# nubomedia/NUBOMEDIA-VCA

Measured on NVIDIA B200. Metric: 1080p face-cascade frames/s, higher is better.
Workload: dtype u8 pixels, int32/u32 integrals, f32 features, f64 stage sums

## Files before the change

nubomedia-vca_b200/csrc/context.cu:

```cuda
#include <math.h>
#include <stdio.h>
#include <stdlib.h>
#include <string.h>

#include <algorithm>
#include <atomic>

#include "internal.h"

#define NV_VERSION_STR "nubovca-b200 0.1 (sm_100a)"
#define CAND_CAP 8192
#define CAND_CAP_GROUPED 65536
#define CAND_CAP_RAW 131072

extern "C" const char *nv_version(void) { return NV_VERSION_STR; }

extern "C" int nv_device_count(void)
{
    int n = 0;
    if (cudaGetDeviceCount(&n) != cudaSuccess) { cudaGetLastError(); return 0; }
    return n;
}

extern "C" int nv_cascade_load(const char *xml_path, nv_cascade **out)
// ... 89 lines not shown
    }
    if (leaves) for (int i = 0; i <= nn; i++) leaves[i] = c->h.leaves[l0 + i];
    return NV_OK;
}

extern "C" int nv_debug_cascade_feature(const nv_cascade *c, int feature, int rects12[12], float weights3[3], int *tilted)
{
    if (!c || feature < 0 || feature >= (int)c->h.feat_tilted.size() || !rects12 || !weights3) { nv_set_error("bad argument"); return NV_ERR_ARG; }
    for (int i = 0; i < 12; i++) rects12[i] = c->h.feat_rect[(size_t)feature * 12 + i];
    for (int i = 0; i < 3; i++) weights3[i] = c->h.feat_weight[(size_t)feature * 3 + i];
    if (tilted) *tilted = c->h.feat_tilted[feature];
    return NV_OK;
}

extern "C" int nv_debug_cascade_subset(const nv_cascade *c, int node, int subset8[8])
{
    if (!c || !subset8 || !c->h.lbp || node < 0 || (size_t)node * 8 + 8 > c->h.node_subset.size()) { nv_set_error("bad argument"); return NV_ERR_ARG; }
    for (int k = 0; k < 8; k++) subset8[k] = c->h.node_subset[(size_t)node * 8 + k];
    return NV_OK;
}

extern "C" void nv_cascade_free(nv_cascade *c)
{
    if (!c) return;
    for (auto &kv : c->d_stumps) { cudaSetDevice(kv.first); cudaFree(kv.second); }
    for (auto &kv : c->d_meta) { cudaSetDevice(kv.first); cudaFree(kv.second); }
    for (auto &kv : c->d_tail) { cudaSetDevice(kv.first); cudaFree(kv.second); }
    for (auto &kv : c->d_tail_base) { cudaSetDevice(kv.first); cudaFree(kv.second); }
    for (auto &kv : c->d_gen) {
        cudaSetDevice(kv.first);
        cudaFree((void *)kv.second.tree); cudaFree((void *)kv.second.node); cudaFree((void *)kv.second.leaf); cudaFree((void *)kv.second.feat);
        cudaFree((void *)kv.second.subset);
    }
    delete c;
}

static int cascade_on_device(nv_cascade *c, int gpu, cudaStream_t st, const DevStump **stumps, const DevCascade **meta)
{
    std::lock_guard<std::mutex> lk(c->mu);
    (void)st;
    if (c->d_stumps.find(gpu) == c->d_stumps.end()) {
        std::vector<void *> owned;
        struct Guard {
            std::vector<void *> &v; bool keep = false;
            ~Guard() { if (!keep) for (void *p : v) cudaFree(p); }
        } guard{owned};
        auto upload = [&](const void *src, size_t bytes, void **out) -> int {
            void *d = nullptr;
            NV_CUDA(cudaMalloc(&d, bytes ? bytes : 1));
            owned.push_back(d);
            if (bytes) NV_CUDA(cudaMemcpy(d, src, bytes, cudaMemcpyHostToDevice));
            *out = d;
            return NV_OK;
        };
        int rc;
        void *ds = nullptr, *dm = nullptr, *dtree = nullptr, *dnode = nullptr, *dleaf = nullptr, *dfeat = nullptr, *dt = nullptr, *db = nullptr, *dsub = nullptr;
        if ((rc = upload(c->stumps.data(), c->stumps.size() * sizeof(DevStump), &ds)) != NV_OK) return rc;
        if ((rc = upload(&c->meta, sizeof(DevCascade), &dm)) != NV_OK) return rc;
        if (c->h.general) {
            const HostCascade &h = c->h;
            std::vector<int2> trees(h.tree_nnodes.size());
            std::vector<int4> nodes(h.node_feat.size());
            std::vector<GenFeat> feats(h.feat_tilted.size());
            int n0 = 0, l0 = 0;
            for (size_t t = 0; t < trees.size(); t++) { trees[t] = make_int2(n0, l0); n0 += h.tree_nnodes[t]; l0 += h.tree_nnodes[t] + 1; }
            for (size_t i = 0; i < nodes.size(); i++) {
                int tb; memcpy(&tb, &h.node_thr[i], 4);
                nodes[i] = make_int4(h.node_feat[i], tb, h.node_left[i], h.node_right[i]);
            }
            for (size_t f = 0; f < feats.size(); f++) {
                GenFeat &g = feats[f];
                memset(&g, 0, sizeof g);
                for (int k = 0; k < 3; k++) {
                    const int *r = &h.feat_rect[f * 12 + 4 * k];
                    g.r[k] = (uint32_t)r[0] | ((uint32_t)r[1] << 8) | ((uint32_t)r[2] << 16) | ((uint32_t)r[3] << 24);
                    g.w[k] = h.feat_weight[f * 3 + k];
                }
                g.tilted = h.feat_tilted[f];
            }
            if ((rc = upload(trees.data(), trees.size() * sizeof(int2), &dtree)) != NV_OK) return rc;
            if ((rc = upload(nodes.data(), nodes.size() * sizeof(int4), &dnode)) != NV_OK) return rc;
            if ((rc = upload(h.leaves.data(), h.leaves.size() * sizeof(float), &dleaf)) != NV_OK) return rc;
            if ((rc = upload(feats.data(), feats.size() * sizeof(GenFeat), &dfeat)) != NV_OK) return rc;
            if (h.lbp && (rc = upload(h.node_subset.data(), h.node_subset.size() * sizeof(int), &dsub)) != NV_OK) return rc;
        }
        if (c->tail_fast) {
            if ((rc = upload(c->tail_stumps.data(), c->tail_stumps.size() * sizeof(TailStump), &dt)) != NV_OK) return rc;
            if ((rc = upload(c->tail_base.data(), c->tail_base.size() * sizeof(double), &db)) != NV_OK) return rc;
        }
        guard.keep = true;
        if (c->h.general) c->d_gen[gpu] = GenModel{(int2 *)dtree, (int4 *)dnode, (float *)dleaf, (GenFeat *)dfeat, (uint32_t *)dsub};
        if (c->tail_fast) { c->d_tail[gpu] = (TailStump *)dt; c->d_tail_base[gpu] = (double *)db; }
        c->d_meta[gpu] = (DevCascade *)dm;
        c->d_stumps[gpu] = (DevStump *)ds;
    }
    *stumps = c->d_stumps[gpu]; *meta = c->d_meta[gpu];
    return NV_OK;
}

template <typename T>
static int ensure(T **p, size_t *cap, size_t need, bool zero = false)
{
    if (*p && *cap >= need) return NV_OK;
    if (*p) { NV_CUDA(cudaFree(*p)); *p = nullptr; }
    size_t n = need + need / 8 + 64;
    NV_CUDA(cudaMalloc(p, n * sizeof(T)));
    if (zero) NV_CUDA(cudaMemset(*p, 0, n * sizeof(T)));
    *cap = n;
    return NV_OK;
}

static int alloc_candidates(nv_ctx *c, int cap, bool with_adj)
{
    cudaFree(c->d_cand); cudaFree(c->d_cand_sorted); cudaFree(c->d_cand_rects); cudaFree(c->d_adj); cudaFree(c->d_result);
    cudaFree(c->d_cand_w); cudaFree(c->d_cls_wmax);
    cudaFreeHost(c->h_result);
    c->d_cand = c->d_cand_sorted = nullptr; c->d_cand_rects = nullptr; c->d_adj = nullptr; c->d_result = c->h_result = nullptr;
    c->d_cand_w = nullptr; c->d_cls_wmax = nullptr;
    c->cand_cap = cap; c->result_cap = cap; c->adj_cap = 0; c->epoch++;
    NV_CUDA(cudaMalloc(&c->d_cand, (size_t)cap * sizeof(uint32_t)));
    NV_CUDA(cudaMalloc(&c->d_cand_sorted, (size_t)cap * sizeof(uint32_t)));
    NV_CUDA(cudaMalloc(&c->d_cand_rects, (size_t)cap * sizeof(int4)));
    NV_CUDA(cudaMalloc(&c->d_cand_w, (size_t)cap * sizeof(double)));
    NV_CUDA(cudaMalloc(&c->d_cls_wmax, (size_t)cap * sizeof(unsigned long long)));
    const size_t acap = std::min<size_t>((size_t)cap, NV_GROUP_UF_MIN);
    size_t adj_words = (with_adj ? acap * ((acap + 31) / 32) : 0) + 8 * (size_t)cap;
    NV_CUDA(cudaMalloc(&c->d_adj, adj_words * sizeof(uint32_t)));
    c->adj_cap = with_adj ? cap : 0;
    c->d_grp = reinterpret_cast<int *>(c->d_adj + (adj_words - 8 * (size_t)cap));
    size_t rbytes = sizeof(ResultHeader) + (size_t)c->result_cap * (sizeof(nv_rect) + sizeof(double) + sizeof(int));
    NV_CUDA(cudaMalloc(&c->d_result, rbytes));
    NV_CUDA(cudaMallocHost(&c->h_result, rbytes));
    memset(c->h_result, 0, sizeof(ResultHeader));
    return NV_OK;
}

extern "C" int nv_ctx_create(int gpu, int max_width, int max_height, nv_ctx **out)
{
    if (!out || max_width <= 0 || max_height <= 0 || max_width > 16384 || max_height > 16384) {
        nv_set_error("nv_ctx_create: bad argument");
        return NV_ERR_ARG;
    }
    *out = nullptr;
    int ndev = nv_device_count();
    if (ndev <= 0) { nv_set_error("no CUDA device visible: libnubovca has no CPU path"); return NV_ERR_NO_DEVICE; }
    if (gpu < 0 || gpu >= ndev) { nv_set_error("gpu ordinal %d out of range (0..%d)", gpu, ndev - 1); return NV_ERR_ARG; }
    NV_CUDA(cudaSetDevice(gpu));
    nv_ctx *c = new nv_ctx();
    c->gpu = gpu; c->max_w = max_width; c->max_h = max_height;
    int rc = [&]() -> int {
        NV_CUDA(cudaStreamCreateWithFlags(&c->stream, cudaStreamNonBlocking));
        NV_CUDA(cudaEventCreateWithFlags(&c->ev_done, cudaEventDisableTiming));
        NV_CUDA(cudaStreamCreateWithFlags(&c->stream2, cudaStreamNonBlocking));
        for (int i = 0; i < 2; i++) {
            NV_CUDA(cudaEventCreateWithFlags(&c->ev_fork[i], cudaEventDisableTiming));
            NV_CUDA(cudaEventCreateWithFlags(&c->ev_join[i], cudaEventDisableTiming));
        }
        c->frame_cap = (size_t)max_width * max_height * 4 + 4096;
        NV_CUDA(cudaMallocHost(&c->h_frame, c->frame_cap));
        NV_CUDA(cudaMalloc(&c->d_frame, c->frame_cap));
        c->gray_cap = (size_t)max_width * max_height + 256;
        NV_CUDA(cudaMalloc(&c->d_gray, c->gray_cap));
        NV_CUDA(cudaMalloc(&c->d_hist, 260 * sizeof(int)));
        NV_CUDA(cudaMemset(c->d_hist, 0, 260 * sizeof(int)));
        NV_CUDA(cudaMalloc(&c->d_lut, 512));
        uint8_t ident[256];
        for (int i = 0; i < 256; i++) ident[i] = (uint8_t)i;
        NV_CUDA(cudaMemcpy(c->d_lut + 256, ident, 256, cudaMemcpyHostToDevice));
        c->slots = new PlanSlot[NV_PLAN_SLOTS];
        c->ps = &c->slots[0];
        for (int i = 0; i < NV_PLAN_SLOTS; i++) NV_CUDA(cudaMalloc(&c->slots[i].d_plan, sizeof(PlanDev)));
        NV_CUDA(cudaMalloc(&c->d_counters, 16 * sizeof(int)));
        NV_CUDA(cudaMemset(c->d_counters, 0, 16 * sizeof(int)));
        NV_CUDA(cudaMalloc(&c->d_deepq, NV_DEEPQ_CAP * sizeof(uint2)));
        return alloc_candidates(c, CAND_CAP, true);
    }();
    if (rc != NV_OK) { nv_ctx_destroy(c); return rc; }
    *out = c;
    return NV_OK;
}

static void batch_free(nv_ctx::Batch &b);

extern "C" void nv_ctx_destroy(nv_ctx *c)
{
    if (!c) return;
    cudaSetDevice(c->gpu);
    if (c->stream) cudaStreamSynchronize(c->stream);
    cudaFreeHost(c->h_frame); cudaFree(c->d_frame); cudaFree(c->d_gray); cudaFree(c->d_hist); cudaFree(c->d_lut);
    cudaFree(c->d_aux); for (auto &e : c->rtabs) cudaFree(e.d); cudaFree(c->d_sum);
    if (c->slots) {
        for (int i = 0; i < NV_PLAN_SLOTS; i++) {
            PlanSlot &sl = c->slots[i];
            cudaFree(sl.d_plan); cudaFree(sl.d_ptab); cudaFree(sl.d_maps);
            if (sl.dexec) cudaGraphExecDestroy(sl.dexec);
        }
        delete[] c->slots;
    }
    cudaFree(c->d_sq); cudaFree(c->d_pyr); cudaFree(c->d_tilt); cudaFree(c->d_vnf); cudaFree(c->d_depth);
    cudaFree(c->d_bits_ok); cudaFree(c->d_queue); cudaFree(c->d_queue2); cudaFree(c->d_deepq); cudaFree(c->d_counters); cudaFree(c->d_cand);
    cudaFree(c->d_cand_sorted); cudaFree(c->d_cand_rects); cudaFree(c->d_adj); cudaFree(c->d_result);
    cudaFree(c->d_cand_w); cudaFree(c->d_cls_wmax);
    cudaFreeHost(c->h_result);
    cudaFree(c->d_trk_prev); cudaFree(c->d_trk_hist); cudaFree(c->d_trk_scratch); cudaFreeHost(c->h_trk);
    if (c->gexec) cudaGraphExecDestroy(c->gexec);
    if (c->bexec) cudaGraphExecDestroy(c->bexec);
    batch_free(c->b);
    if (c->ev_done) cudaEventDestroy(c->ev_done);
    for (int i = 0; i < 2; i++) { if (c->ev_fork[i]) cudaEventDestroy(c->ev_fork[i]); if (c->ev_join[i]) cudaEventDestroy(c->ev_join[i]); }
    if (c->stream2) cudaStreamDestroy(c->stream2);
    for (int i = 0; i <= NV_NUM_STAGES; i++) if (c->prof_ev[i]) cudaEventDestroy(c->prof_ev[i]);
    if (c->stream) cudaStreamDestroy(c->stream);
    cudaGetLastError();
    delete c;
}

extern "C" int nv_ctx_set_scores(nv_ctx *ctx, int on)
{
    if (!ctx) { nv_set_error("null ctx"); return NV_ERR_ARG; }
    ctx->scores = on ? 1 : 0;
    return NV_OK;
}

extern "C" int nv_get_scores(nv_ctx *ctx, int *neighbors, double *level_weights, int cap, int *n)
{
    if (!ctx) { nv_set_error("null ctx"); return NV_ERR_ARG; }
    if (!ctx->scores_ready || ctx->batch_last) { nv_set_error("no collected call with scores on"); return NV_ERR_STATE; }
    const int total = reinterpret_cast<const ResultHeader *>(ctx->h_result)->n_out, m = std::min(total, std::max(cap, 0));
    const uint8_t *w = ctx->h_result + sizeof(ResultHeader) + (size_t)ctx->result_cap * sizeof(nv_rect);
    const uint8_t *nb = w + (size_t)ctx->result_cap * sizeof(double);
    if (level_weights && m > 0) memcpy(level_weights, w, (size_t)m * sizeof(double));
    if (neighbors && m > 0) memcpy(neighbors, nb, (size_t)m * sizeof(int));
    if (n) *n = m;
    if (total > cap) { nv_set_error("%d rectangles, caller capacity %d", total, cap); return NV_ERR_CAPACITY; }
    return NV_OK;
}

extern "C" int nv_ctx_set_debug(nv_ctx *ctx, int debug)
{
    if (!ctx) { nv_set_error("null ctx"); return NV_ERR_ARG; }
    ctx->debug = debug ? 1 : 0;
    ctx->epoch++;
    for (int i = 0; ctx->slots && i < NV_PLAN_SLOTS; i++) ctx->slots[i].plan_valid = false;
    return NV_OK;
}

static const char *k_stage_names[NV_NUM_STAGES] = {"face_prep", "hist_lut", "pyramid_rowscan", "integral_colscan",
                                                   "cascade_stage0", "cascade_tiles", "cascade_tail", "group_rectangles"};
extern "C" const char *nv_stage_name(int slot) { return slot >= 0 && slot < NV_NUM_STAGES ? k_stage_names[slot] : ""; }

static inline void prof_mark(nv_ctx *ctx, int idx)
{
    if (!ctx->profile) return;
    cudaStreamCaptureStatus cs = cudaStreamCaptureStatusNone;
    cudaStreamIsCapturing(ctx->stream, &cs);
    if (cs == cudaStreamCaptureStatusActive) cudaEventRecordWithFlags(ctx->prof_ev[idx], ctx->stream, cudaEventRecordExternal);
    else cudaEventRecord(ctx->prof_ev[idx], ctx->stream);
    ctx->prof_set[idx] = true;
}

extern "C" int nv_ctx_set_profile(nv_ctx *ctx, int on)
{
    if (!ctx) { nv_set_error("null ctx"); return NV_ERR_ARG; }
    NV_CUDA(cudaSetDevice(ctx->gpu));
    if (on && !ctx->prof_ev[0])
        for (int i = 0; i <= NV_NUM_STAGES; i++) NV_CUDA(cudaEventCreate(&ctx->prof_ev[i]));
    if (ctx->profile != (on ? 1 : 0)) ctx->epoch++;
    ctx->profile = on ? 1 : 0;
    return NV_OK;
}

extern "C" int nv_ctx_get_stage_times(nv_ctx *ctx, float *ms, int cap, int *n)
{
    if (!ctx || !ms) { nv_set_error("null argument"); return NV_ERR_ARG; }
    if (!ctx->profile || ctx->pending) { nv_set_error("profiling off or call still pending"); return NV_ERR_STATE; }
    if (ctx->batch_last) { nv_set_error("stage times describe single calls: the last call was a batch"); return NV_ERR_STATE; }
    NV_CUDA(cudaSetDevice(ctx->gpu));
    int m = std::min(cap, NV_NUM_STAGES);
    for (int i = 0; i < m; i++) {
        ms[i] = 0.f;
        if (ctx->prof_set[i] && ctx->prof_set[i + 1]) NV_CUDA(cudaEventElapsedTime(&ms[i], ctx->prof_ev[i], ctx->prof_ev[i + 1]));
    }
    if (n) *n = m;
    return NV_OK;
}

extern "C" int nv_event_create(void **ev)
{
    if (!ev) { nv_set_error("null argument"); return NV_ERR_ARG; }
    cudaEvent_t e;
    NV_CUDA(cudaEventCreate(&e));
    *ev = e;
    return NV_OK;
}
extern "C" int nv_event_record(nv_ctx *ctx, void *ev)
{
    if (!ctx || !ev) { nv_set_error("null argument"); return NV_ERR_ARG; }
    NV_CUDA(cudaSetDevice(ctx->gpu));
    NV_CUDA(cudaEventRecord((cudaEvent_t)ev, ctx->stream));
    return NV_OK;
}
extern "C" int nv_event_elapsed_ms(void *e0, void *e1, float *ms)
{
    if (!e0 || !e1 || !ms) { nv_set_error("null argument"); return NV_ERR_ARG; }
    NV_CUDA(cudaEventSynchronize((cudaEvent_t)e1));
    NV_CUDA(cudaEventElapsedTime(ms, (cudaEvent_t)e0, (cudaEvent_t)e1));
    return NV_OK;
}
extern "C" void nv_event_destroy(void *ev) { if (ev) cudaEventDestroy((cudaEvent_t)ev); }

static inline int cv_round(double v) { return (int)lrint(v); }
static inline int cv_roundf(float v) { return (int)lrintf(v); }
static inline int align_up(int v, int a) { return (v + a - 1) / a * a; }

static void exact_coefs(int ssize, int dsize, int2 *tab, int lead, int total)
{
    double scale = 1.0 / ((double)dsize / ssize);
    for (int k = 0; k < total; k++) tab[k] = make_int2(0, 0);
    for (int d = 0; d < dsize; d++) {
        double f = scale * (d + 0.5) - 0.5;
        int i = (int)floor(f);
        if (i >= 0 && i < ssize - 1) tab[lead + d] = make_int2(i, cv_round((f - i) * 256.0));
        else if (i < 0) tab[lead + d] = make_int2(0, 0);
        else tab[lead + d] = ssize >= 2 ? make_int2(ssize - 2, 256) : make_int2(0, 0);
    }
}

static int ensure_plan(nv_ctx *ctx, const nv_cascade *casc, int W, int H, const nv_detect_params *p)
{
    if (!(p->scale_factor > 1.0)) {
        nv_set_error("scale_factor must be > 1 (got %g): OpenCV would never terminate", p->scale_factor);
        return NV_ERR_ARG;
    }
    PlanKey key;
    key.W = W; key.H = H; key.win_w = casc->h.win_w; key.win_h = casc->h.win_h;
    key.min_w = p->min_w; key.min_h = p->min_h; key.max_w = p->max_w; key.max_h = p->max_h; key.sf = p->scale_factor;
    key.casc = casc->uid;
    if (ctx->ps->plan_valid && key == ctx->ps->pkey) { ctx->ps->last_use = ++ctx->use_clock; return NV_OK; }
    PlanSlot *victim = nullptr;
    for (int i = 0; i < NV_PLAN_SLOTS; i++) {
        PlanSlot &sl = ctx->slots[i];
        if (sl.plan_valid && key == sl.pkey) {
            ctx->ps = &sl;
            sl.last_use = ++ctx->use_clock;
            if (sl.buf_gen != ctx->buf_gen) { sl.tp_casc = 0; sl.buf_gen = ctx->buf_gen; }
            return NV_OK;
        }
        if (!victim || (!sl.plan_valid && victim->plan_valid) || (sl.plan_valid == victim->plan_valid && sl.last_use < victim->last_use))
            victim = &sl;
    }
    ctx->ps = victim;
    ctx->ps->plan_valid = false;
    ctx->ps->last_use = ++ctx->use_clock;

    PlanDev &P = ctx->ps->plan;
    memset(&P, 0, sizeof P);
    P.W = W; P.H = H; P.win_w = key.win_w; P.win_h = key.win_h;
    int max_w = p->max_w, max_h = p->max_h;
    if (max_w == 0 || max_h == 0) { max_w = W; max_h = H; }
    std::vector<float> scales;
    for (double f = 1;; f *= p->scale_factor) {
        int ww = cv_round(key.win_w * f), wh = cv_round(key.win_h * f);
        if (ww > max_w || wh > max_h || ww > W || wh > H) break;
        if (ww < p->min_w || wh < p->min_h) continue;
        scales.push_back((float)f);
        if (scales.size() > 4096) break;
    }
    int nstripes = 1;
    long long iofs = 0, wofs = 0, bofs = 0, tofs = 0, pofs = 0;
    int nl = 0;
    for (size_t k = 0; k < scales.size(); k++) {
        float sc = scales[k];
        int lw = cv_roundf((float)W / sc), lh = cv_roundf((float)H / sc);
        int rx = lw + 1 - key.win_w, ry = lh + 1 - key.win_h;
        if (k == 0) nstripes = std::max((std::max(rx, 0) + 31) / 32, 1);
        if (rx <= 0 || ry <= 0) continue;
        int ystep = sc >= 2.f ? 1 : 2;
        int stripe = std::max((ry / ystep + nstripes - 1) / nstripes, 1) * ystep;
        long long lim = (long long)stripe * nstripes;
        if (lim < ry) ry = (int)lim;
        if (nl >= NV_MAX_LEVELS) { nv_set_error("more than %d pyramid levels", NV_MAX_LEVELS); return NV_ERR_CAPACITY; }
        LevelDesc &L = P.lv[nl++];
        L.scale = sc; L.lw = lw; L.lh = lh; L.ystep = ystep;
        L.nx = (rx + ystep - 1) / ystep; L.ny = (ry + ystep - 1) / ystep; L.nxw = (L.nx + 31) / 32;
        if (L.nx > 8191 || L.ny > 8191) { nv_set_error("level too large for 13-bit window ids"); return NV_ERR_CAPACITY; }
        L.iplane = align_up((lw + 1 + ystep - 1) / ystep, 4);
        L.ipitch = L.iplane * ystep;
        L.iofs = (int)iofs; iofs += (long long)L.ipitch * (lh + 1);
        L.wofs = (int)wofs; wofs += (long long)L.nx * L.ny;
        L.bofs = (int)bofs; bofs += (long long)L.nxw * L.ny;
        L.xtab = (int)tofs; L.ytab = (int)tofs + align_up(lw + 1, 4); tofs += align_up(lw + 1, 4) + align_up(lh, 2);
        L.pofs = (int)pofs; pofs += (long long)lw * lh;
        L.rowblk0 = P.total_rowblk; P.total_rowblk += (lh + 7) / 8;
        L.colblk0 = P.total_colblk; P.total_colblk += (L.ipitch + NV_COLBLK - 1) / NV_COLBLK;
        L.chunk0 = P.total_chunks; P.total_chunks += L.nxw * L.ny;
        L.row0 = P.total_rows; P.total_rows += L.ny;
        L.dblk0 = P.total_dblk; P.total_dblk += (lw + lh + 255) / 256;
        L.cntx = (L.nx + NV_CTX - 1) / NV_CTX;
        int cnt = L.cntx * ((L.ny + NV_CTY - 1) / NV_CTY);
        if (ystep == 2) { L.ctile0 = P.ctiles2; P.ctiles2 += cnt; P.nlv2 = nl; }
        else { L.ctile0 = P.ctiles1; P.ctiles1 += cnt; }
        L.wtile0 = 0; L.wntx = 0;
        if (ystep == 1) {
            L.wntx = (L.nx + NV_WTX - 1) / NV_WTX;
            L.wtile0 = P.wtiles[1]; P.wtiles[1] += L.wntx * ((L.ny + NV_WTY - 1) / NV_WTY);
        }
        if (iofs > 0x7fffffffLL || wofs > 0x7fffffffLL) { nv_set_error("frame too large"); return NV_ERR_CAPACITY; }
    }
    P.nlevels = nl;
    P.total_windows = (int)wofs;

    NV_CUDA(cudaStreamSynchronize(ctx->stream));
    if (nl > 0) {
        std::vector<int2> tab((size_t)tofs);
        for (int l = 0; l < nl; l++) {
            exact_coefs(W, P.lv[l].lw, &tab[P.lv[l].xtab], 1, align_up(P.lv[l].lw + 1, 4));
            exact_coefs(H, P.lv[l].lh, &tab[P.lv[l].ytab], 0, align_up(P.lv[l].lh, 2));
        }
        int rc;
        if ((rc = ensure(&ctx->ps->d_ptab, &ctx->ps->ptab_cap, (size_t)tofs * 2)) != NV_OK) return rc;
        NV_CUDA(cudaMemcpy(ctx->ps->d_ptab, tab.data(), (size_t)tofs * sizeof(int2), cudaMemcpyHostToDevice));
        const void *old[8] = {ctx->d_sum, ctx->d_sq, ctx->d_vnf, ctx->d_queue, ctx->d_bits_ok, ctx->d_depth, ctx->d_pyr, ctx->d_tilt};
        struct MovedGuard {
            nv_ctx *c; const void *const *old;
            ~MovedGuard()
            {
                const void *now[8] = {c->d_sum, c->d_sq, c->d_vnf, c->d_queue, c->d_bits_ok, c->d_depth, c->d_pyr, c->d_tilt};
                if (memcmp(old, now, sizeof now)) { c->buf_gen++; c->epoch++; }
            }
        } moved_guard{ctx, old};
        size_t icap = ctx->integ_cap;
        if ((rc = ensure(&ctx->d_sum, &icap, (size_t)iofs, true)) != NV_OK) return rc;
        if ((rc = ensure(&ctx->d_sq, &ctx->integ_cap, (size_t)iofs, true)) != NV_OK) return rc;
        size_t wcap = ctx->win_cap;
        if ((rc = ensure(&ctx->d_vnf, &wcap, (size_t)wofs)) != NV_OK) return rc;
        if ((rc = ensure(&ctx->d_queue, &ctx->queue_cap, (size_t)wofs)) != NV_OK) return rc;
        ctx->win_cap = wcap;
        if ((rc = ensure(&ctx->d_bits_ok, &ctx->bits_cap, (size_t)bofs * 3)) != NV_OK) return rc;
        ctx->ps->bits_words = bofs;
        if (ctx->debug) {
            if ((rc = ensure(&ctx->d_depth, &ctx->depth_cap, (size_t)wofs)) != NV_OK) return rc;
            if ((rc = ensure(&ctx->d_pyr, &ctx->pyr_cap, (size_t)pofs)) != NV_OK) return rc;
        }
        if (ctx->need_tilt && (rc = ensure(&ctx->d_tilt, &ctx->tilt_cap, ctx->integ_cap)) != NV_OK) return rc;
        ctx->ps->max_lw = 0;
        for (int l = 0; l < nl; l++) ctx->ps->max_lw = std::max(ctx->ps->max_lw, P.lv[l].lw);
    }
    NV_CUDA(cudaMemcpy(ctx->ps->d_plan, &P, sizeof(PlanDev), cudaMemcpyHostToDevice));
    ctx->ps->pkey = key;
    ctx->ps->plan_valid = true;
    ctx->ps->tp_casc = 0;
    ctx->ps->buf_gen = ctx->buf_gen;
    ctx->ps->gen++;
    if (ctx->ps->dexec) { cudaGraphExecDestroy(ctx->ps->dexec); ctx->ps->dexec = nullptr; }
    ctx->ps->dkey = DetGraphKey(); ctx->ps->dkey_seen = DetGraphKey();
    return NV_OK;
}

typedef CUresult (*encode_tiled_fn)(CUtensorMap *, CUtensorMapDataType, cuuint32_t, void *, const cuuint64_t *,
                                    const cuuint64_t *, const cuuint32_t *, const cuuint32_t *, CUtensorMapInterleave,
                                    CUtensorMapSwizzle, CUtensorMapL2promotion, CUtensorMapFloatOOBfill);

static encode_tiled_fn get_encode_tiled()
{
    static encode_tiled_fn fn = []() -> encode_tiled_fn {
        void *p = nullptr;
        cudaDriverEntryPointQueryResult q;
        if (cudaGetDriverEntryPoint("cuTensorMapEncodeTiled", &p, cudaEnableDefault, &q) != cudaSuccess ||
            q != cudaDriverEntryPointSuccess) { cudaGetLastError(); return nullptr; }
        return (encode_tiled_fn)p;
    }();
    return fn;
}

static int ensure_tile_params(nv_ctx *ctx, const nv_cascade *casc)
{
    if (ctx->ps->tp_casc == casc->uid) return NV_OK;
    const PlanDev &P = ctx->ps->plan;
    const DevCascade &m = casc->meta;
    ctx->ps->tp_casc = casc->uid;
    ctx->ps->use_tiles = false;  ctx->ps->use_s0t = false;
    ctx->ps->gen++;
    if (ctx->ps->dexec) { cudaGraphExecDestroy(ctx->ps->dexec); ctx->ps->dexec = nullptr; }
    ctx->ps->use_s0p = !casc->h.general && P.nlevels > 0 && fill_stage0_params(casc, P, &ctx->ps->s0p);
    encode_tiled_fn enc = get_encode_tiled();
    if (casc->h.general || !enc || m.win_w > 32 || m.win_h > 32 || P.nlevels == 0) return NV_OK;
    int end = 1;
    while (end < m.nstages && end < NV_BULK_MAX_STAGES && m.stage_first[end + 1] - m.stage_first[1] <= NV_BULK_MAX_STUMPS) end++;
    ctx->ps->bulk_end = end;
    static_assert(sizeof(CUtensorMap) == 128, "tensor map size");
    alignas(64) CUtensorMap maps[2 * NV_MAX_LEVELS];
    memset(maps, 0, sizeof maps);
    if (!ctx->ps->d_maps) NV_CUDA(cudaMalloc(&ctx->ps->d_maps, sizeof maps));
    for (int c = 0; c < 2; c++) {
        int ys = c == 0 ? 2 : 1;
        TileParams &tp = ctx->ps->tp[c];
        struct Geo { int cp, rt, ps, kskew; };
        auto geometry = [&](int tw, int th) {
            Geo g;
            g.cp = align_up(tw + (ys == 2 ? m.win_w / 2 : m.win_w) + 1, 4);
            if (g.cp % 8 == 0) g.cp += 4;
            g.rt = (th - 1) * ys + m.win_h + 1;
            g.kskew = (ys * g.cp) & 31;
            g.ps = align_up(g.rt * g.cp, 32);
            return g;
        };
        const Geo g0 = geometry(NV_CTX, NV_CTY);
        const Geo g = ys == 1 ? geometry(NV_WTX, NV_WTY) : g0;
        if (g.cp > 256 || g.rt > 256) return NV_OK;
        tp.cp = g.cp; tp.rt = g.rt; tp.kskew = g.kskew; tp.ps = g.ps;
        tp.level_begin = c == 0 ? 0 : P.nlv2;
        tp.level_end = c == 0 ? P.nlv2 : P.nlevels;
        fill_bulk_stumps(casc, ys, tp.cp, tp.ps, 1, end, &tp);
        Stage0TileParams &s0 = ctx->ps->s0t[c];
        const bool s0ok = tp.fast && fill_stage0_tile_params(casc, ys, g0.cp, g0.rt, g0.ps, g0.kskew, &s0);
        ctx->ps->use_s0t = c == 0 ? s0ok : (ctx->ps->use_s0t && s0ok);
        s0.level_begin = tp.level_begin; s0.level_end = tp.level_end;
        for (int l = tp.level_begin; l < tp.level_end; l++) {
            const LevelDesc &L = P.lv[l];
            cuuint64_t gdim[2] = {(cuuint64_t)L.ipitch, (cuuint64_t)(L.lh + 1)};
            cuuint64_t gstr[1] = {(cuuint64_t)L.ipitch * 4};
            cuuint32_t estr[2] = {1, 1};
            for (int k = 0; k < 2; k++) {
                cuuint32_t box[2] = {(cuuint32_t)(k == 0 ? g.cp : g0.cp), (cuuint32_t)(k == 0 ? g.rt : g0.rt)};
                CUresult r = enc(&maps[k * NV_MAX_LEVELS + l], CU_TENSOR_MAP_DATA_TYPE_UINT32, 2, ctx->d_sum + L.iofs, gdim, gstr, box, estr,
                                 CU_TENSOR_MAP_INTERLEAVE_NONE, CU_TENSOR_MAP_SWIZZLE_NONE, CU_TENSOR_MAP_L2_PROMOTION_L2_128B,
                                 CU_TENSOR_MAP_FLOAT_OOB_FILL_NONE);
                if (r != CUDA_SUCCESS) return NV_OK;
            }
        }
    }
    NV_CUDA(cudaStreamSynchronize(ctx->stream));
    NV_CUDA(cudaMemcpy(ctx->ps->d_maps, maps, sizeof maps, cudaMemcpyHostToDevice));
    ctx->ps->use_tiles = true;
    return NV_OK;
}

static int detect_prepare(nv_ctx *ctx, nv_cascade *casc, int W, int H, const nv_detect_params *p)
{
    int rc = ensure_plan(ctx, casc, W, H, p);
    if (rc != NV_OK) return rc;
    if ((rc = cascade_on_device(casc, ctx->gpu, ctx->stream, &ctx->cur_stumps, &ctx->cur_meta)) != NV_OK) return rc;
    ctx->cur_tail = nullptr; ctx->cur_tail_base = nullptr;
    ctx->use_gen = casc->h.general != 0;
    if (ctx->use_gen) {
        std::lock_guard<std::mutex> lk(casc->mu);
        ctx->cur_gen = casc->d_gen[ctx->gpu];
    }
    ctx->cur_tilted = casc->h.has_tilted != 0;
    if (ctx->cur_tilted) {
        if (!ctx->need_tilt || ctx->tilt_cap < ctx->integ_cap) {
            NV_CUDA(cudaStreamSynchronize(ctx->stream));
            ctx->need_tilt = true;
            if ((rc = ensure(&ctx->d_tilt, &ctx->tilt_cap, ctx->integ_cap)) != NV_OK) return rc;
            ctx->epoch++; ctx->buf_gen++;
        }
    }
    if (casc->tail_fast) {
        std::lock_guard<std::mutex> lk(casc->mu);
        ctx->cur_tail = casc->d_tail[ctx->gpu]; ctx->cur_tail_base = casc->d_tail_base[ctx->gpu];
    }
    if (ctx->use_gen && ctx->ps->plan.total_windows > NV_SMALL_PLAN_WINDOWS && ctx->queue2_cap < ctx->queue_cap) {
        NV_CUDA(cudaStreamSynchronize(ctx->stream));
        if ((rc = ensure(&ctx->d_queue2, &ctx->queue2_cap, ctx->queue_cap)) != NV_OK) return rc;
        ctx->epoch++; ctx->buf_gen++;
    }
    if ((rc = ensure_tile_params(ctx, casc)) != NV_OK) return rc;
    if (p->min_neighbors > 0 && ctx->adj_cap < (size_t)ctx->cand_cap) {
        NV_CUDA(cudaStreamSynchronize(ctx->stream));
        if ((rc = alloc_candidates(ctx, std::min(ctx->cand_cap, CAND_CAP_GROUPED), true)) != NV_OK) return rc;
    }
    return NV_OK;
}

static int detect_enqueue(nv_ctx *ctx, nv_cascade *casc, const uint8_t *d_gray, int W, int H, int gstride,
                          const uint8_t *d_lut, const nv_detect_params *p, int *nlaunch)
{
    const DevStump *stumps = ctx->cur_stumps;
    const DevCascade *meta = ctx->cur_meta;
    const PlanDev &P = ctx->ps->plan;
    cudaStream_t st = ctx->stream;
    int nl = 0;
    for (int i = 2; i <= NV_NUM_STAGES; i++) ctx->prof_set[i] = false;
    struct CountersGuard {
        nv_ctx *c; cudaStream_t s; bool done = false;
        ~CountersGuard() { if (!done) { cudaMemsetAsync(c->d_counters, 0, 16 * sizeof(int), s); cudaGetLastError(); } }
    } counters_guard{ctx, st};
    if (P.nlevels > 0) {
        int16_t *depth = ctx->debug ? ctx->d_depth : nullptr;
        prof_mark(ctx, 2);
        const uint32_t *tilt = ctx->use_gen && ctx->cur_tilted ? ctx->d_tilt : nullptr;
        NV_CUDA(launch_pyr_rowscan(ctx->ps->d_plan, P.total_rowblk, d_gray, gstride, d_lut, ctx->ps->d_ptab, ctx->d_sum, ctx->d_sq,
                                   ctx->debug ? ctx->d_pyr : nullptr, st));
        prof_mark(ctx, 3);
        NV_CUDA(launch_colscan(ctx->ps->d_plan, P.total_colblk, ctx->d_sum, ctx->d_sq, st));
        if (tilt) { NV_CUDA(launch_tilted(ctx->ps->d_plan, P.total_dblk, ctx->d_sum, ctx->d_tilt, st)); nl += 2; }
        prof_mark(ctx, 4);
        const bool small_fast = ctx->ps->use_tiles && ctx->cur_tail && P.total_windows <= NV_SMALL_PLAN_WINDOWS && casc->meta.nstages > 1;
        const int qcap = (int)std::min<size_t>(ctx->queue_cap, 0x7fffffff);
        bool queued = false;
        if (ctx->use_gen) {
            NV_CUDA(launch_stage0_rows_gen(ctx->ps->d_plan, P.total_rows, meta, ctx->cur_gen, ctx->d_sum, ctx->d_sq, tilt, ctx->d_vnf,
                                           ctx->d_bits_ok, ctx->d_counters, depth, st));
        } else if (ctx->ps->use_tiles && ctx->ps->use_s0t && P.total_windows > NV_SMALL_PLAN_WINDOWS) {
            uint32_t *bits_fail = ctx->d_bits_ok + ctx->ps->bits_words, *bits_okv = ctx->d_bits_ok + 2 * (size_t)ctx->ps->bits_words;
            const bool fork = P.ctiles2 > 0 && P.ctiles1 > 0;
            if (fork) { NV_CUDA(cudaEventRecord(ctx->ev_fork[0], st)); NV_CUDA(cudaStreamWaitEvent(ctx->stream2, ctx->ev_fork[0], 0)); }
            for (int c = 0; c < 2; c++) {
                Stage0TileParams &s0 = ctx->ps->s0t[c];
                int ntiles = c == 0 ? P.ctiles2 : P.ctiles1;
                if (ntiles == 0) continue;
                s0.maps = ctx->ps->d_maps + NV_MAX_LEVELS; s0.plan = ctx->ps->d_plan; s0.sq = ctx->d_sq; s0.vnf = ctx->d_vnf;
                s0.bits_fail = bits_fail; s0.bits_okv = bits_okv;
                NV_CUDA(launch_stage0_tiles(s0, c == 0 ? 2 : 1, ntiles, c == 1 && fork ? ctx->stream2 : st));
                nl++;
            }
            if (fork) { NV_CUDA(cudaEventRecord(ctx->ev_join[0], ctx->stream2)); NV_CUDA(cudaStreamWaitEvent(st, ctx->ev_join[0], 0)); }
            NV_CUDA(launch_stage0_chain(P, bits_fail, bits_okv, ctx->d_bits_ok, ctx->d_counters, depth, st));
        } else if (ctx->ps->use_s0p) {
            Stage0Params &sp = ctx->ps->s0p;
            sp.sum = ctx->d_sum; sp.sq = ctx->d_sq; sp.vnf = ctx->d_vnf; sp.bits_alive = ctx->d_bits_ok;
            sp.counters = ctx->d_counters; sp.depth = depth;
            sp.queue = small_fast ? ctx->d_queue : nullptr; sp.queue_cap = qcap; sp.queue_cidx = 3;
            queued = small_fast;
            NV_CUDA(launch_stage0_rows_p(sp, st));
        } else
            NV_CUDA(launch_stage0_rows(ctx->ps->d_plan, P.total_rows, meta, stumps, ctx->d_sum, ctx->d_sq, ctx->d_vnf,
                                       ctx->d_bits_ok, ctx->d_counters, depth, st));
        prof_mark(ctx, 5);
        nl += 3;
        if (small_fast) {
            if (!queued) {
                NV_CUDA(launch_alive_to_queue(ctx->ps->d_plan, P.total_rows, ctx->d_vnf, ctx->d_bits_ok, ctx->d_queue, ctx->d_counters,
                                              qcap, st, 3));
                nl++;
            }
            prof_mark(ctx, 6);
            int split = 1;
            while (split < casc->meta.nstages && casc->meta.stage_first[split + 1] - casc->meta.stage_first[split] < NV_TAIL_BLOCK_MIN_STUMPS) split++;
            if (tail_tab_smem(casc->meta, 1, casc->meta.nstages) <= NV_TAILTAB_MAX_SMEM) split = casc->meta.nstages;
            if (tail_tab_smem(casc->meta, 1, split) <= NV_TAILTAB_MAX_SMEM)
                NV_CUDA(launch_cascade_tail_tab(ctx->ps->d_plan, meta, casc->meta, ctx->cur_tail, ctx->cur_tail_base, ctx->d_sum, ctx->d_queue,
                                                ctx->d_counters, ctx->d_cand, ctx->cand_cap, depth, 1, split, ctx->d_deepq, NV_DEEPQ_CAP, st));
            else
                NV_CUDA(launch_cascade_tail_fast(ctx->ps->d_plan, meta, ctx->cur_tail, ctx->cur_tail_base, ctx->d_sum, ctx->d_queue,
                                                 ctx->d_counters, ctx->d_cand, ctx->cand_cap, depth, 1, split, ctx->d_deepq, NV_DEEPQ_CAP, st,
                                                 8 * (casc->meta.win_w + 1) * (casc->meta.win_h + 1) * 4));
            nl += 1;
            if (split < casc->meta.nstages) {
                NV_CUDA(launch_cascade_tail_block(ctx->ps->d_plan, meta, ctx->cur_tail, ctx->cur_tail_base, ctx->d_sum, ctx->d_deepq,
                                                  ctx->d_counters, 6, ctx->d_cand, ctx->cand_cap, depth, split, -1, st));
                nl++;
            }
        } else if (ctx->ps->use_tiles) {
            const bool fork = P.ctiles2 > 0 && P.ctiles1 > 0;
            if (fork) { NV_CUDA(cudaEventRecord(ctx->ev_fork[1], st)); NV_CUDA(cudaStreamWaitEvent(ctx->stream2, ctx->ev_fork[1], 0)); }
            for (int c = 0; c < 2; c++) {
                TileParams &tp = ctx->ps->tp[c];
                const cudaStream_t cst = c == 1 && fork ? ctx->stream2 : st;
                if ((c == 0 ? P.ctiles2 : P.ctiles1) == 0) continue;
                tp.plan = ctx->ps->d_plan; tp.bits_alive = ctx->d_bits_ok; tp.vnf = ctx->d_vnf; tp.depth = depth;
                tp.tail = ctx->d_queue; tp.cand = ctx->d_cand; tp.counters = ctx->d_counters; tp.maps = ctx->ps->d_maps;
                tp.tail_cap = qcap; tp.cand_cap = ctx->cand_cap;
                if (c == 0) NV_CUDA(launch_cascade_classes(tp, P.ctiles2, cst));
                else NV_CUDA(launch_cascade_wide(tp, P.wtiles[1], cst));
                nl++;
            }
            if (fork) { NV_CUDA(cudaEventRecord(ctx->ev_join[1], ctx->stream2)); NV_CUDA(cudaStreamWaitEvent(st, ctx->ev_join[1], 0)); }
            prof_mark(ctx, 6);
            if (ctx->ps->bulk_end < casc->meta.nstages && ctx->cur_tail) {
                NV_CUDA(launch_cascade_tail_fast(ctx->ps->d_plan, meta, ctx->cur_tail, ctx->cur_tail_base, ctx->d_sum, ctx->d_queue,
                                                 ctx->d_counters, ctx->d_cand, ctx->cand_cap, depth, ctx->ps->bulk_end, casc->meta.nstages,
                                                 nullptr, qcap, st, 8 * (casc->meta.win_w + 1) * (casc->meta.win_h + 1) * 4));
                nl++;
            } else if (ctx->ps->bulk_end < casc->meta.nstages) {
                NV_CUDA(launch_cascade_tail(ctx->ps->d_plan, meta, stumps, ctx->d_sum, ctx->d_queue, ctx->d_counters, ctx->d_cand,
                                            ctx->cand_cap, depth, ctx->ps->bulk_end, casc->h.order_free, 148 * 8, st,
                                            8 * (casc->meta.win_w + 1) * (casc->meta.win_h + 1) * 4));
                nl++;
            }
        } else {
            NV_CUDA(launch_alive_to_queue(ctx->ps->d_plan, P.total_rows, ctx->d_vnf, ctx->d_bits_ok, ctx->d_queue, ctx->d_counters,
                                          qcap, st));
            prof_mark(ctx, 6);
            if (ctx->use_gen && P.total_windows > NV_SMALL_PLAN_WINDOWS && ctx->d_queue2 && ctx->queue2_cap >= ctx->queue_cap && casc->meta.nstages > 1) {
                int extra = 0;
                NV_CUDA(launch_queue_stages_gen_staged(ctx->ps->d_plan, meta, ctx->cur_gen, ctx->d_sum, tilt, ctx->d_queue, ctx->d_queue2, qcap,
                                                       ctx->d_counters, ctx->d_cand, ctx->cand_cap, depth, casc->meta.nstages,
                                                       casc->h.order_free, st, &extra));
                nl += extra - 1;
            } else if (ctx->use_gen)
                NV_CUDA(launch_queue_stages_gen(ctx->ps->d_plan, meta, ctx->cur_gen, ctx->d_sum, tilt, ctx->d_queue, ctx->d_counters,
                                                ctx->d_cand, ctx->cand_cap, depth, 148 * 8, casc->h.order_free, st));
            else
                NV_CUDA(launch_queue_stages(ctx->ps->d_plan, meta, stumps, ctx->d_sum, ctx->d_queue, ctx->d_counters, ctx->d_cand,
                                            ctx->cand_cap, depth, 148 * 8, st));
            nl += 2;
        }
    }
    prof_mark(ctx, 7);
    const ScoreArgs sa = {ctx->cur_meta, ctx->cur_stumps, ctx->use_gen ? ctx->cur_gen : GenModel{}, ctx->use_gen ? 1 : 0, ctx->d_sum, ctx->d_sq,
                          ctx->use_gen && ctx->cur_tilted ? ctx->d_tilt : nullptr, ctx->d_cand_w, ctx->d_cls_wmax};
    NV_CUDA(launch_group(ctx->ps->d_plan, ctx->d_counters, ctx->d_cand, ctx->cand_cap, ctx->d_cand_sorted, ctx->d_cand_rects,
                         ctx->d_adj, ctx->d_grp, p->min_neighbors, 0.2, W, H, ctx->d_result, ctx->result_cap, 148 * 2, st, &nl,
                         P.total_windows <= NV_SMALL_PLAN_WINDOWS, ctx->h_result, ctx->scores ? &sa : nullptr));
    prof_mark(ctx, 8);
    *nlaunch += nl;
    counters_guard.done = true;
    return NV_OK;
}

static void detect_bookkeeping(nv_ctx *ctx, nv_cascade *casc, const uint8_t *d_gray, int W, int H, int gstride,
                               const uint8_t *d_lut, const nv_detect_params *p)
{
    ctx->last_min_neighbors = p->min_neighbors;
    ctx->last_casc = casc; ctx->last_params = *p; ctx->last_W = W; ctx->last_H = H;
    ctx->tap_gray = d_gray; ctx->tap_lut = d_lut; ctx->tap_stride = gstride;
    ctx->last_scores = ctx->scores != 0; ctx->scores_ready = false;
    ctx->pending = true;
    ctx->batch_last = false;
}

int nv_detect_device(nv_ctx *ctx, nv_cascade *casc, const uint8_t *d_gray, int W, int H, int gstride,
                     const uint8_t *d_lut, const nv_detect_params *p)
{
    int rc = detect_prepare(ctx, casc, W, H, p);
    if (rc != NV_OK) return rc;
    PlanSlot *sl = ctx->ps;
    DetGraphKey key;
    key.gray = d_gray; key.gstride = gstride; key.lut = d_lut; key.casc = casc->uid; key.sf = p->scale_factor; key.mn = p->min_neighbors;
    key.epoch = ctx->epoch; key.scores = ctx->scores;
    bool graphable = !ctx->debug && !ctx->profile && !ctx->no_graph;
    int nl = 0;
    if (graphable && sl->dexec && key == sl->dkey) {
        NV_CUDA(cudaGraphLaunch(sl->dexec, ctx->stream));
        nl = sl->d_nl;
    } else if (graphable && key == sl->dkey_seen) {
        if (sl->dexec) { cudaGraphExecDestroy(sl->dexec); sl->dexec = nullptr; }
        cudaGraph_t g = nullptr;
        NV_CUDA(cudaStreamBeginCapture(ctx->stream, cudaStreamCaptureModeThreadLocal));
        rc = detect_enqueue(ctx, casc, d_gray, W, H, gstride, d_lut, p, &nl);
        cudaError_t ce = cudaStreamEndCapture(ctx->stream, &g);
        if (rc != NV_OK || ce != cudaSuccess || !g) {
            if (g) cudaGraphDestroy(g);
            cudaGetLastError();
            ctx->no_graph = true;
            nl = 0;
            if ((rc = detect_enqueue(ctx, casc, d_gray, W, H, gstride, d_lut, p, &nl)) != NV_OK) return rc;
        } else {
            ce = cudaGraphInstantiate(&sl->dexec, g, 0);
            cudaGraphDestroy(g);
            if (ce != cudaSuccess) { sl->dexec = nullptr; nv_set_error("cudaGraphInstantiate: %s", cudaGetErrorString(ce)); return NV_ERR_CUDA; }
            sl->dkey = key; sl->d_nl = nl;
            NV_CUDA(cudaGraphLaunch(sl->dexec, ctx->stream));
        }
    } else {
        sl->dkey_seen = key;
        if ((rc = detect_enqueue(ctx, casc, d_gray, W, H, gstride, d_lut, p, &nl)) != NV_OK) return rc;
    }
    ctx->launches += nl;
    detect_bookkeeping(ctx, casc, d_gray, W, H, gstride, d_lut, p);
    return NV_OK;
}

int nv_collect(nv_ctx *ctx, nv_rect *out, int cap, int *n)
{
    if (!ctx->pending) { nv_set_error("collect without a pending submit"); return NV_ERR_STATE; }
    NV_CUDA(cudaStreamSynchronize(ctx->stream));
    ctx->pending = false;
    const ResultHeader *h = reinterpret_cast<const ResultHeader *>(ctx->h_result);
    if (h->overflow) {
        int need = h->n_cand, lim = ctx->last_min_neighbors > 0 ? CAND_CAP_GROUPED : CAND_CAP_RAW;
        if (need > lim || need <= ctx->cand_cap) {
            nv_set_error("%d raw candidates exceed the supported maximum of %d", need, lim);
            return NV_ERR_CAPACITY;
        }
        int rc = alloc_candidates(ctx, std::min(lim, need + need / 4 + 64), ctx->last_min_neighbors > 0);
        if (rc != NV_OK) return rc;
        nv_detect_params p = ctx->last_params;
        const int scores = ctx->scores;
        ctx->scores = ctx->last_scores;
        rc = nv_detect_device(ctx, ctx->last_casc, ctx->tap_gray, ctx->last_W, ctx->last_H, ctx->tap_stride, ctx->tap_lut, &p);
        ctx->scores = scores;
        if (rc != NV_OK) return rc;
        NV_CUDA(cudaStreamSynchronize(ctx->stream));
        ctx->pending = false;
        h = reinterpret_cast<const ResultHeader *>(ctx->h_result);
    }
    int total = h->n_out;
    if (total > NV_RESULT_INLINE) {
        NV_CUDA(cudaMemcpy(ctx->h_result + sizeof(ResultHeader) + NV_RESULT_INLINE * sizeof(nv_rect),
                           ctx->d_result + sizeof(ResultHeader) + NV_RESULT_INLINE * sizeof(nv_rect),
                           (size_t)(total - NV_RESULT_INLINE) * sizeof(nv_rect), cudaMemcpyDeviceToHost));
        if (ctx->last_scores) {
            const size_t wofs = sizeof(ResultHeader) + (size_t)ctx->result_cap * sizeof(nv_rect), nofs = wofs + (size_t)ctx->result_cap * sizeof(double);
            NV_CUDA(cudaMemcpy(ctx->h_result + wofs + NV_RESULT_INLINE * sizeof(double), ctx->d_result + wofs + NV_RESULT_INLINE * sizeof(double),
                               (size_t)(total - NV_RESULT_INLINE) * sizeof(double), cudaMemcpyDeviceToHost));
            NV_CUDA(cudaMemcpy(ctx->h_result + nofs + NV_RESULT_INLINE * sizeof(int), ctx->d_result + nofs + NV_RESULT_INLINE * sizeof(int),
                               (size_t)(total - NV_RESULT_INLINE) * sizeof(int), cudaMemcpyDeviceToHost));
        }
    }
    ctx->scores_ready = ctx->last_scores;
    int m = std::min(total, cap);
    if (out && m > 0) memcpy(out, ctx->h_result + sizeof(ResultHeader), (size_t)m * sizeof(nv_rect));
    if (n) *n = m;
    if (h->overflow) {
        nv_set_error("internal capacity exceeded (%d raw candidates, cap %d)", h->n_cand, ctx->cand_cap);
        return NV_ERR_CAPACITY;
    }
    if (total > cap) { nv_set_error("%d rectangles, caller capacity %d", total, cap); return NV_ERR_CAPACITY; }
    return NV_OK;
}

int nv_h2d(nv_ctx *ctx, const uint8_t *src, size_t bytes)
{
    cudaPointerAttributes at;
    bool known = cudaPointerGetAttributes(&at, src) == cudaSuccess;
    if (known && (at.type == cudaMemoryTypeDevice || at.type == cudaMemoryTypeManaged)) {
        NV_CUDA(cudaMemcpyAsync(ctx->d_frame, src, bytes, cudaMemcpyDeviceToDevice, ctx->stream));
        return NV_OK;
    }
// ... 1016 lines not shown
```

nubomedia-vca_b200/csrc/internal.h:

```cpp
#pragma once
#include <cuda.h>
#include <cuda_runtime.h>
#include <stdint.h>

#include <map>
#include <mutex>
#include <string>
#include <vector>

#include "nubovca.h"

#define NV_GROUP_UF_MIN 2048
#define NV_SMALL_PLAN_WINDOWS 16384
#define NV_DEEPQ_CAP NV_SMALL_PLAN_WINDOWS
#define NV_TAILTAB_MAX_SMEM (200 * 1024)
#define NV_TAIL_BLOCK_MIN_STUMPS 64
#define NV_COLBLK 128
#define NV_MAX_LEVELS 64
#define NV_MAX_STAGES 64
#define NV_RESULT_INLINE 1024
#define NV_HIST_STRIDE 260
#define NV_BATCH_GROUP_CAP NV_RESULT_INLINE

void nv_set_error(const char *fmt, ...);
#define NV_CUDA(call)                                                                        \
    do {                                                                                     \
        cudaError_t e_ = (call);                                                             \
        if (e_ != cudaSuccess) {                                                             \
            nv_set_error("%s failed: %s (%s:%d)", #call, cudaGetErrorString(e_), __FILE__, __LINE__); \
            return NV_ERR_CUDA;                                                              \
        }                                                                                    \
    } while (0)

struct HostCascade {
    int win_w = 0, win_h = 0;
    std::vector<int> stage_ntrees;
    std::vector<float> stage_thr;
    std::vector<int> stump_feat;
    std::vector<float> stump_thr, stump_left, stump_right;
    std::vector<int> feat_rect;
    std::vector<float> feat_weight;
    int n3rect = 0;
    int order_free = 0;
    int general = 0, has_tilted = 0;
    std::vector<int> tree_nnodes;
    std::vector<int> node_feat, node_left, node_right;
    std::vector<float> node_thr, leaves;
    std::vector<uint8_t> feat_tilted;
    int lbp = 0;
    std::vector<int> node_subset;
};

int nv_parse_cascade_xml(const char *path, HostCascade *out);

struct __align__(16) DevStump {
    uint32_t r[3];
    float w[3];
    float thr, left, right;
    uint32_t pad[3];
};

struct __align__(16) GenFeat {
    uint32_t r[3];
    float w[3];
    int tilted;
    int pad;
};
struct GenModel {
    const int2 *tree;
    const int4 *node;
    const float *leaf;
    const GenFeat *feat;
    const uint32_t *subset;
};

struct DevCascade {
    int win_w, win_h, nstages, nstumps;
    int stage_first[NV_MAX_STAGES + 1];
    float stage_thr[NV_MAX_STAGES];
};

struct __align__(16) TailStump {
    uint16_t o[12];
    float thr;
    int16_t w1, w2;
    double d128;
    uint32_t pad[2];
};
static_assert(sizeof(TailStump) == 48, "three 16-byte loads");

struct nv_cascade {
    unsigned long long uid = 0;
    HostCascade h;
    std::vector<DevStump> stumps;
    DevCascade meta;
    int tail_fast = 0;
    std::vector<TailStump> tail_stumps;
    std::vector<double> tail_base;
    std::mutex mu;
    std::map<int, DevStump *> d_stumps;
    std::map<int, DevCascade *> d_meta;
    std::map<int, TailStump *> d_tail;
    std::map<int, double *> d_tail_base;
    std::map<int, GenModel> d_gen;
};

struct LevelDesc {
    float scale;
    int lw, lh;
    int ystep;
    int nx, ny, nxw;
    int ipitch;
    int iplane;
    int iofs;
    int wofs;
    int bofs;
    int xtab, ytab;
    int pofs;
    int rowblk0;
    int colblk0;
    int chunk0;
    int row0;
    int dblk0;
    int ctile0, cntx;
    int wtile0, wntx;
};

struct PlanDev {
    int nlevels;
    int W, H;
    int win_w, win_h;
    int total_rowblk, total_colblk, total_chunks, total_rows, total_windows;
    int nlv2;
    int ctiles2, ctiles1;
    int wtiles[2];
    int total_dblk;
    LevelDesc lv[NV_MAX_LEVELS];
};

struct PlanKey {
    int W = 0, H = 0, win_w = 0, win_h = 0, min_w = 0, min_h = 0, max_w = 0, max_h = 0;
    double sf = 0;
    unsigned long long casc = 0;
    bool operator==(const PlanKey &o) const {
        return W == o.W && H == o.H && win_w == o.win_w && win_h == o.win_h && min_w == o.min_w &&
               min_h == o.min_h && max_w == o.max_w && max_h == o.max_h && sf == o.sf && casc == o.casc;
    }
};

struct ResizeKey {
    int sw = 0, sh = 0, dw = 0, dh = 0;
    bool operator==(const ResizeKey &o) const { return sw == o.sw && sh == o.sh && dw == o.dw && dh == o.dh; }
};

#define NV_BULK_MAX_STUMPS 384
#define NV_BULK_MAX_STAGES 16
#define NV_CTX 64
#define NV_CTY 32
#define NV_WTX 128
#define NV_WTY 64

struct __align__(16) BulkStump {
    uint4 o0, o1;
    uint32_t w0, w1, w2, thr;
    uint32_t d_lo, d_hi;
    uint32_t left, right;
};

struct TileParams {
    BulkStump s[NV_BULK_MAX_STUMPS];
    uint4 o2[NV_BULK_MAX_STUMPS];
    int stage_first[NV_BULK_MAX_STAGES + 1];
    int stage_mid6[NV_BULK_MAX_STAGES];
    int stage_mid[NV_BULK_MAX_STAGES];
    float stage_thr[NV_BULK_MAX_STAGES];
    double stage_base[NV_BULK_MAX_STAGES];
    int stage_begin, stage_end;
    int final_stage;
    int fast;
    int level_begin, level_end;
    int cp, rt, ps;
    int kskew;
    const CUtensorMap *maps;
    const PlanDev *plan;
    const uint32_t *bits_alive;
    const float *vnf;
    int16_t *depth;
    uint2 *tail;
    uint32_t *cand;
    int *counters;
    int tail_cap, cand_cap;
};
static_assert(sizeof(TileParams) <= 32000, "kernel parameter space is 32764 bytes");

#define NV_S0T_MAX_STUMPS 8
struct Stage0TileParams {
    BulkStump s[NV_S0T_MAX_STUMPS];
    uint4 o2[NV_S0T_MAX_STUMPS];
    int stage_first[2], stage_mid6[1], stage_mid[1];
    float stage_thr[1];
    double stage_base[1];
    uint4 var;
    int win_w, win_h;
    int level_begin, level_end;
    int cp, rt, ps, kskew;
    const CUtensorMap *maps;
    const PlanDev *plan;
    const uint32_t *sq;
    float *vnf;
    uint32_t *bits_fail, *bits_okv;
};

#define NV_S0_MAX_STUMPS 8
struct Stage0Params {
    uint4 off[NV_MAX_LEVELS][NV_S0_MAX_STUMPS][3];
    int4 var[NV_MAX_LEVELS];
    int4 lv_a[NV_MAX_LEVELS];
    int4 lv_b[NV_MAX_LEVELS];
    float2 cf[NV_S0_MAX_STUMPS][3];
    int nlevels, total_rows, n0, win_w, win_h;
    float thr0;
    const uint32_t *sum, *sq;
    float *vnf;
    uint32_t *bits_alive;
    int *counters;
    int16_t *depth;
    uint2 *queue;
    int queue_cap, queue_cidx;
    size_t integ_stride;
    int win_stride, bits_stride;
};
static_assert(sizeof(Stage0Params) <= 32000, "kernel parameter space is 32764 bytes");

struct ResultHeader {
    int n_out;
    int n_cand;
    int n_alive;
    int overflow;
};

struct DetGraphKey {
    const void *gray = nullptr; int gstride = 0; const void *lut = nullptr; unsigned long long casc = 0;
    double sf = 0; int mn = 0; unsigned long long epoch = 0; int scores = 0;
    bool operator==(const DetGraphKey &o) const {
        return gray == o.gray && gstride == o.gstride && lut == o.lut && casc == o.casc && sf == o.sf && mn == o.mn && epoch == o.epoch &&
               scores == o.scores;
    }
};
struct PlanSlot {
    PlanKey pkey;  bool plan_valid = false;
    PlanDev plan;
    PlanDev *d_plan = nullptr;
    int *d_ptab = nullptr;       size_t ptab_cap = 0;
    Stage0TileParams s0t[2];  bool use_s0t = false;  int bits_words = 0;
    TileParams tp[2];  Stage0Params s0p;  bool use_s0p = false;  CUtensorMap *d_maps = nullptr;  bool use_tiles = false;
    int bulk_end = 0;  unsigned long long tp_casc = 0;  int max_lw = 0;
    unsigned long long last_use = 0, buf_gen = 0;
    unsigned long long gen = 0;
    cudaGraphExec_t dexec = nullptr;  DetGraphKey dkey, dkey_seen;  int d_nl = 0;
};
#define NV_PLAN_SLOTS 12

struct TrkLayout { int ntx, nty; size_t bbox, rects, out, bseed, parent, slotlist, bcount, keys, bslot, counters, edge_flag, zero_begin, zero_end; };

struct nv_ctx {
    int gpu = 0;
    int max_w = 0, max_h = 0;
    int debug = 0;
    cudaStream_t stream = nullptr;
    cudaEvent_t ev_done = nullptr;
    cudaStream_t stream2 = nullptr;
    cudaEvent_t ev_fork[2] = {}, ev_join[2] = {};

    uint8_t *h_frame = nullptr;  size_t frame_cap = 0;
    uint8_t *d_frame = nullptr;
    uint8_t *d_gray = nullptr;   size_t gray_cap = 0;
    int *d_hist = nullptr;
    uint8_t *d_lut = nullptr;
    uint8_t *d_aux = nullptr;    size_t aux_cap = 0;

    struct RtabEntry { ResizeKey k; int *d = nullptr; int row_a = 0, row_period = 0; };
    RtabEntry rtabs[16];  int rtab_next = 0;

    PlanSlot *slots = nullptr;  PlanSlot *ps = nullptr;  unsigned long long use_clock = 0, buf_gen = 1;
    uint32_t *d_sum = nullptr, *d_sq = nullptr;  size_t integ_cap = 0;
    uint8_t *d_pyr = nullptr;    size_t pyr_cap = 0;
    float *d_vnf = nullptr;      size_t win_cap = 0;
    int16_t *d_depth = nullptr;  size_t depth_cap = 0;
    uint32_t *d_bits_ok = nullptr;  size_t bits_cap = 0;
    uint2 *d_queue = nullptr;    size_t queue_cap = 0;
    int *d_counters = nullptr;
    uint32_t *d_cand = nullptr;  int cand_cap = 0;
    uint32_t *d_cand_sorted = nullptr;
    int4 *d_cand_rects = nullptr;
    uint32_t *d_adj = nullptr;   size_t adj_cap = 0;  int *d_grp = nullptr;
    uint8_t *d_result = nullptr; uint8_t *h_result = nullptr;
    int result_cap = 0;
    int scores = 0;  bool last_scores = false, scores_ready = false;
    double *d_cand_w = nullptr;  unsigned long long *d_cls_wmax = nullptr;

    struct GraphKey {
        const void *src = nullptr; int w = 0, h = 0, stride = 0, cols = 0, rows = 0; const int *rtab = nullptr;
        unsigned long long casc = 0; double sf = 0; int mn = 0, min_w = 0, min_h = 0; unsigned long long epoch = 0;
        const PlanSlot *slot = nullptr; unsigned long long slot_gen = 0;
        int fmt = 0; const void *p1 = nullptr, *p2 = nullptr; int s1 = 0, s2 = 0;
        int scores = 0;
        bool operator==(const GraphKey &o) const {
            return scores == o.scores && fmt == o.fmt && p1 == o.p1 && p2 == o.p2 && s1 == o.s1 && s2 == o.s2 && src == o.src && w == o.w && h == o.h && stride == o.stride && cols == o.cols && rows == o.rows &&
                   rtab == o.rtab && casc == o.casc && sf == o.sf && mn == o.mn && min_w == o.min_w && min_h == o.min_h &&
                   epoch == o.epoch && slot == o.slot && slot_gen == o.slot_gen;
        }
    };
    const DevStump *cur_stumps = nullptr;  const DevCascade *cur_meta = nullptr;
    const TailStump *cur_tail = nullptr;  const double *cur_tail_base = nullptr;
    GenModel cur_gen = {};  bool use_gen = false;  bool cur_tilted = false;
    bool need_tilt = false;
    uint2 *d_queue2 = nullptr;  size_t queue2_cap = 0;
    uint2 *d_deepq = nullptr;
    uint32_t *d_tilt = nullptr;  size_t tilt_cap = 0;
    cudaGraphExec_t gexec = nullptr;  GraphKey gkey, gkey_seen;  int g_nl = 0;  bool no_graph = false;  unsigned g_prof_mask = 0;
    unsigned long long epoch = 1;

    nv_cascade *last_casc = nullptr;  nv_detect_params last_params = {};  int last_W = 0, last_H = 0;
    const uint8_t *tap_gray = nullptr, *tap_lut = nullptr;  int tap_stride = 0;
    bool pending = false;
    int profile = 0;  cudaEvent_t prof_ev[NV_NUM_STAGES + 1] = {};  bool prof_set[NV_NUM_STAGES + 1] = {};
    int last_min_neighbors = 0;
    long long launches = 0;

    struct Batch {
        int cap = 0;
        size_t frame_bytes = 0, gray_bytes = 0, integ = 0, wins = 0, bits = 0;
        uint8_t *d_frame = nullptr, *h_stage = nullptr;
        uint8_t *d_gray = nullptr, *d_lut = nullptr;  int *d_hist = nullptr;
        uint32_t *d_sum = nullptr, *d_sq = nullptr, *d_bits = nullptr;  float *d_vnf = nullptr;
        uint2 *d_queue = nullptr;  uint32_t *d_cand = nullptr, *d_sorted = nullptr;  int4 *d_rects = nullptr;
        uint32_t *d_adj = nullptr;  int *d_grp = nullptr;
        int *d_counters = nullptr;
        uint8_t *d_result = nullptr, *h_result = nullptr;
        const uint8_t **d_tab = nullptr, **h_tab = nullptr;
        std::vector<const uint8_t *> tab_last;
        unsigned long long gen = 1;
    } b;
    struct BatchKey {
        int kind = 0, n = 0, w = 0, h = 0, stride = 0, cols = 0, rows = 0; const int *rtab = nullptr; bool aligned = false;
        unsigned long long casc = 0; double sf = 0; int mn = 0, min_w = 0, min_h = 0, max_w = 0, max_h = 0;
        unsigned long long epoch = 0, bgen = 0; const PlanSlot *slot = nullptr; unsigned long long slot_gen = 0;
        bool operator==(const BatchKey &o) const {
            return kind == o.kind && n == o.n && w == o.w && h == o.h && stride == o.stride && cols == o.cols && rows == o.rows &&
                   rtab == o.rtab && aligned == o.aligned && casc == o.casc && sf == o.sf && mn == o.mn && min_w == o.min_w &&
                   min_h == o.min_h && max_w == o.max_w && max_h == o.max_h && epoch == o.epoch && bgen == o.bgen && slot == o.slot &&
                   slot_gen == o.slot_gen;
        }
    };
    cudaGraphExec_t bexec = nullptr;  BatchKey bkey, bkey_seen;  int b_nl = 0;
    bool batch_last = false, batch_routed = false, batch_replayed = false;  int batch_n = 0, batch_kind = 0;
    std::vector<const uint8_t *> batch_src;  int batch_w = 0, batch_h = 0, batch_stride = 0;  bool batch_on_device = false;
    nv_face_params batch_fp = {};  nv_detect_params batch_dp = {};  nv_cascade *batch_casc = nullptr;
    long long batch_sum[3] = {0, 0, 0}, batch_launches = 0;
    std::vector<nv_rect> batch_out;  std::vector<int> batch_counts;

    uint8_t *d_trk_prev = nullptr, *d_trk_hist = nullptr, *d_trk_scratch = nullptr;
    TrkLayout trk_lo = {};
    float trk_val[256] = {};
    int trk_w = 0, trk_h = 0;  long long trk_frames = 0;
    uint8_t *h_trk = nullptr;
};

struct SrcPlanes { const uint8_t *p0, *p1, *p2; int s0, s1, s2; };
cudaError_t launch_face_prep_yuv(int fmt, const SrcPlanes &s, int sw, int sh, uint8_t *gray, int dw, int dh, const int *rtab,
                                 int *hist, cudaStream_t st, uint8_t *lut = nullptr);
cudaError_t launch_yuv2bgr(int fmt, const SrcPlanes &s, int w, int h, uint8_t *dst, int dstride, cudaStream_t st);
cudaError_t launch_yuv2gray(int fmt, const SrcPlanes &s, int w, int h, uint8_t *dst, int dstride, cudaStream_t st);
int nv_yuv_upload(nv_ctx *ctx, const nv_yuv_frame *f, SrcPlanes *planes);
cudaError_t launch_face_prep(const uint8_t *src, int sw, int sh, int sstride, int cn, uint8_t *gray, int dw, int dh,
                             const int *rtab, int *hist, cudaStream_t st, uint8_t *lut = nullptr);
cudaError_t launch_bgr2gray(const uint8_t *src, int w, int h, int sstride, int cn, uint8_t *dst, int dstride,
                            cudaStream_t st);
cudaError_t launch_resize_linear(const uint8_t *src, int sw, int sh, int sstride, int cn, uint8_t *dst, int dw, int dh,
                                 int dstride, const int *rtab, cudaStream_t st);
cudaError_t launch_hist(const uint8_t *src, int w, int h, int stride, int *hist, cudaStream_t st, uint8_t *lut = nullptr);
cudaError_t launch_apply_lut(const uint8_t *src, int w, int h, int sstride, const uint8_t *lut, uint8_t *dst, int dstride,
                             cudaStream_t st);
cudaError_t launch_flip(const uint8_t *src, int w, int h, int sstride, uint8_t *dst, int dstride, cudaStream_t st);
void build_resize_tables(int sw, int sh, int dw, int dh, std::vector<int> &tab);
enum { RT_COPY = 0, RT_BOX2 = 1, RT_LINEAR = 2 };

cudaError_t launch_pyr_rowscan(const PlanDev *plan, int total_rowblk, const uint8_t *gray, int gstride, const uint8_t *lut,
                               const int *ptab, uint32_t *sum, uint32_t *sq, uint8_t *pyr_debug, cudaStream_t st);
cudaError_t launch_colscan(const PlanDev *plan, int total_colblk, uint32_t *sum, uint32_t *sq, cudaStream_t st);
cudaError_t launch_tilted(const PlanDev *plan, int total_dblk, const uint32_t *sum, uint32_t *tilt, cudaStream_t st);

cudaError_t launch_queue_stages(const PlanDev *plan, const DevCascade *meta, const DevStump *stumps, const uint32_t *sum,
                                const uint2 *queue, int *counters, uint32_t *cand, int cand_cap, int16_t *depth,
                                int nblocks, cudaStream_t st);

cudaError_t launch_stage0_rows(const PlanDev *plan, int total_rows, const DevCascade *meta, const DevStump *stumps,
                               const uint32_t *sum, const uint32_t *sq, float *vnf, uint32_t *bits_alive, int *counters,
                               int16_t *depth, cudaStream_t st);
cudaError_t launch_stage0_rows_gen(const PlanDev *plan, int total_rows, const DevCascade *meta, const GenModel &g,
                                   const uint32_t *sum, const uint32_t *sq, const uint32_t *tilt, float *vnf,
                                   uint32_t *bits_alive, int *counters, int16_t *depth, cudaStream_t st);
cudaError_t launch_queue_stages_gen(const PlanDev *plan, const DevCascade *meta, const GenModel &g, const uint32_t *sum,
                                    const uint32_t *tilt, const uint2 *queue, int *counters, uint32_t *cand, int cand_cap,
                                    int16_t *depth, int nblocks, int order_free, cudaStream_t st);
cudaError_t launch_queue_stages_gen_staged(const PlanDev *plan, const DevCascade *meta, const GenModel &g, const uint32_t *sum,
                                           const uint32_t *tilt, uint2 *queue_a, uint2 *queue_b, int qcap, int *counters,
                                           uint32_t *cand, int cand_cap, int16_t *depth, int nstages, int order_free,
                                           cudaStream_t st, int *nlaunch);
cudaError_t launch_cascade_classes(const TileParams &tp, int ntiles, cudaStream_t st);
cudaError_t launch_cascade_wide(const TileParams &tp, int ntiles, cudaStream_t st);
cudaError_t launch_stage0_rows_p(const Stage0Params &sp, cudaStream_t st);
bool fill_stage0_params(const nv_cascade *c, const PlanDev &P, Stage0Params *sp);
cudaError_t launch_cascade_tail(const PlanDev *plan, const DevCascade *meta, const DevStump *stumps, const uint32_t *sum,
                                const uint2 *tail, int *counters, uint32_t *cand, int cand_cap, int16_t *depth,
                                int stage_begin, int order_free, int nblocks, cudaStream_t st, int smem_bytes);
cudaError_t launch_alive_to_queue(const PlanDev *plan, int total_rows, const float *vnf, const uint32_t *bits_alive,
                                  uint2 *queue, int *counters, int queue_cap, cudaStream_t st, int cidx = 4);
void fill_bulk_stumps(const nv_cascade *c, int ystep, int cp, int ps, int stage_begin, int stage_end, TileParams *tp);
bool fill_stage0_tile_params(const nv_cascade *c, int ystep, int cp, int rt, int ps, int kskew, Stage0TileParams *sp);
cudaError_t launch_stage0_tiles(const Stage0TileParams &sp, int ystep, int ntiles, cudaStream_t st);
cudaError_t launch_stage0_chain(const PlanDev &plan, const uint32_t *bits_fail, const uint32_t *bits_okv,
                                uint32_t *bits_alive, int *counters, int16_t *depth, cudaStream_t st);
void build_tail_stumps(nv_cascade *c);
cudaError_t launch_cascade_tail_fast(const PlanDev *plan, const DevCascade *meta, const TailStump *tstumps, const double *tbase,
                                     const uint32_t *sum, const uint2 *tail, int *counters, uint32_t *cand, int cand_cap,
                                     int16_t *depth, int stage_begin, int stage_end, uint2 *deep, int deep_cap, cudaStream_t st,
                                     int smem_bytes);
size_t tail_tab_smem(const DevCascade &m, int stage_begin, int stage_end);
cudaError_t launch_cascade_tail_tab(const PlanDev *plan, const DevCascade *meta, const DevCascade &hmeta, const TailStump *tstumps,
                                    const double *tbase, const uint32_t *sum, const uint2 *tail, int *counters, uint32_t *cand,
                                    int cand_cap, int16_t *depth, int stage_begin, int stage_end, uint2 *deep, int deep_cap,
                                    cudaStream_t st);
cudaError_t launch_cascade_tail_block(const PlanDev *plan, const DevCascade *meta, const TailStump *tstumps, const double *tbase,
                                      const uint32_t *sum, const uint2 *queue, int *counters, int cin, uint32_t *cand, int cand_cap,
                                      int16_t *depth, int stage_begin, int skip_counter, cudaStream_t st);

int nv_detect_device(nv_ctx *ctx, nv_cascade *casc, const uint8_t *d_gray, int W, int H, int gstride, const uint8_t *d_lut,
                     const nv_detect_params *p);
int nv_collect(nv_ctx *ctx, nv_rect *out, int cap, int *n);
cudaError_t launch_face_prep_batch(const uint8_t *const *srcs, int n, bool aligned, int sw, int sh, int sstride, uint8_t *gray,
                                   int dw, int dh, const int *rtab, int *hist, uint8_t *lut, cudaStream_t st);
cudaError_t launch_pyramid_batch(const PlanDev *plan, int total_rowblk, int total_colblk, int n, const uint8_t *const *grays, int gstride,
                                 const uint8_t *lut, int lut_stride, const int *ptab, uint32_t *sum, uint32_t *sq, size_t integ_stride,
                                 cudaStream_t st);
cudaError_t launch_stage0_rows_p_batch(const Stage0Params &sp, int n, cudaStream_t st);
cudaError_t launch_cascade_tail_tab_batch(const PlanDev *plan, const DevCascade *meta, const DevCascade &hmeta, const TailStump *tstumps,
                                          const double *tbase, const uint32_t *sum, size_t integ_stride, const uint2 *queue, int queue_cap,
                                          int *counters, uint32_t *cand, int cand_stride, cudaStream_t st);
cudaError_t launch_group_batch(const PlanDev *plan, int n, int *counters, const uint32_t *cand, int cand_stride, int cap, uint32_t *cand_sorted,
                               int4 *cand_rects, uint32_t *adj, size_t adj_stride, int *grp, int min_neighbors, double eps, int img_w,
                               int img_h, uint8_t *result, uint8_t *host_result, size_t result_stride, cudaStream_t st);
int nv_h2d(nv_ctx *ctx, const uint8_t *src, size_t bytes);
int nv_get_rtab(nv_ctx *ctx, int sw, int sh, int dw, int dh, const int **d_tab, const nv_ctx::RtabEntry **entry = nullptr);

struct ScoreArgs {
    const DevCascade *meta;
    const DevStump *stumps;
    GenModel g;
    int general;
    const uint32_t *sum, *sq, *tilt;
    double *w;
    unsigned long long *cls_wmax;
};
cudaError_t launch_group(const PlanDev *plan, int *counters, const uint32_t *cand, int cand_cap, uint32_t *cand_sorted,
                         int4 *cand_rects, uint32_t *adj, int *grp, int min_neighbors, double eps, int img_w, int img_h,
                         uint8_t *result, int result_cap, int nblocks, cudaStream_t st, int *nlaunch, bool fused = false, uint8_t *host_result = nullptr,
                         const ScoreArgs *scores = nullptr);

size_t tracker_scratch_bytes(int w, int h, TrkLayout *lo);
cudaError_t launch_tracker(nv_ctx *ctx, int fmt, const SrcPlanes &src, int w, int h, int first, int thr, int cur, const float *val256,
                           int *nlaunch);

#ifdef __CUDACC__
struct YuvTerms { int b, g, r; };

template <int FMT>
__device__ __forceinline__ YuvTerms yuv_chroma(const SrcPlanes &s, int x, int y)
{
    int u, v;
    if (FMT == 1) {
        u = s.p1[(size_t)(y >> 1) * s.s1 + (x >> 1)];
        v = s.p2[(size_t)(y >> 1) * s.s2 + (x >> 1)];
    } else {
        const uint8_t *uv = s.p1 + (size_t)(y >> 1) * s.s1 + (x & ~1);
        u = uv[FMT == 2 ? 0 : 1];
        v = uv[FMT == 2 ? 1 : 0];
    }
    u -= 128; v -= 128;
    YuvTerms t;
    t.b = (1 << 19) + 2116026 * u;
    t.g = (1 << 19) - 852492 * v - 409993 * u;
    t.r = (1 << 19) + 1673527 * v;
    return t;
}

__device__ __forceinline__ int sat_u8(int v) { return min(max(v, 0), 255); }

__device__ __forceinline__ void yuv_pixel(const SrcPlanes &s, const YuvTerms &t, int x, int y, int c3[3])
{
    int yy = max(0, (int)s.p0[(size_t)y * s.s0 + x] - 16) * 1220542;
    c3[0] = sat_u8((yy + t.b) >> 20);
    c3[1] = sat_u8((yy + t.g) >> 20);
    c3[2] = sat_u8((yy + t.r) >> 20);
}
#endif
```

nubomedia-vca_b200/csrc/kernels_cascade.cu:

```cuda
#include "cascade_eval.cuh"

#include <set>

__device__ __forceinline__ int find_level_c(const PlanDev *__restrict__ plan, int idx, int LevelDesc::*first)
{
    int n = plan->nlevels, l = 0;
    while (l + 1 < n && plan->lv[l + 1].*first <= idx) l++;
    return l;
}

__device__ __forceinline__ int uniformize_s0(int v)
{
    int r = 0;
    for (int k = 0; k < 3; k++) r |= (int)(__ballot_sync(0xffffffffu, (v >> k) & 1) & (1u << k));
    return r;
}

__global__ void __launch_bounds__(256)
k_queue_stages(const PlanDev *__restrict__ plan, const DevCascade *__restrict__ meta, const DevStump *__restrict__ stumps,
               const uint32_t *__restrict__ sum, const uint2 *__restrict__ queue, int *__restrict__ counters,
               uint32_t *__restrict__ cand, int cand_cap, int16_t *__restrict__ depth)
{
    int n = counters[0];
    int nstages = meta->nstages;
// ... 380 lines not shown

__global__ void __launch_bounds__(256)
k_alive_to_queue(const PlanDev *__restrict__ plan, int total_rows, const float *__restrict__ vnf,
                 const uint32_t *__restrict__ bits_alive, uint2 *__restrict__ queue, int *__restrict__ counters,
                 int queue_cap, int cidx)
{
    int lane = threadIdx.x & 31;
    int row = blockIdx.x * 8 + (threadIdx.x >> 5);
    if (row >= total_rows) return;
    int l = find_level_c(plan, row, &LevelDesc::row0);
    const LevelDesc &L = plan->lv[l];
    int iy = row - L.row0;
    for (int cx = 0; cx < L.nxw; cx++) {
        uint32_t am = bits_alive[L.bofs + iy * L.nxw + cx];
        if (!am) continue;
        int base = 0;
        if (lane == 0) base = atomicAdd(&counters[cidx], __popc(am));
        base = __shfl_sync(0xffffffffu, base, 0);
        if ((am >> lane) & 1u) {
            int ix = cx * 32 + lane, pos = base + __popc(am & ((1u << lane) - 1u));
            if (pos < queue_cap)
                queue[pos] = make_uint2(((uint32_t)l << 26) | ((uint32_t)iy << 13) | (uint32_t)ix,
                                        __float_as_uint(vnf[L.wofs + iy * L.nx + ix]));
            else
                counters[2] = 1;
        }
    }
}

__device__ __forceinline__ uint32_t smem_u32(const void *p) { return (uint32_t)__cvta_generic_to_shared(p); }

__device__ __forceinline__ void mbar_init(uint32_t bar, uint32_t count)
{
    asm volatile("mbarrier.init.shared::cta.b64 [%0], %1;" ::"r"(bar), "r"(count));
    asm volatile("fence.mbarrier_init.release.cluster;" ::: "memory");
}
__device__ __forceinline__ void mbar_expect_tx(uint32_t bar, uint32_t bytes)
{
    asm volatile("mbarrier.arrive.expect_tx.shared::cta.b64 _, [%0], %1;" ::"r"(bar), "r"(bytes) : "memory");
}
__device__ __forceinline__ void mbar_wait(uint32_t bar, uint32_t phase)
{
    uint32_t done;
    do {
        asm volatile("{\n\t.reg .pred p;\n\tmbarrier.try_wait.parity.shared::cta.b64 p, [%1], %2;\n\tselp.u32 %0, 1, 0, p;\n\t}"
                     : "=r"(done) : "r"(bar), "r"(phase) : "memory");
    } while (!done);
}
__device__ __forceinline__ void tma_load_2d(uint32_t dst, const CUtensorMap *map, int x, int y, uint32_t bar)
{
    asm volatile("cp.async.bulk.tensor.2d.shared::cluster.global.mbarrier::complete_tx::bytes [%0], [%1, {%3, %4}], [%2];"
                 ::"r"(dst), "l"(reinterpret_cast<uint64_t>(map)), "r"(bar), "r"(x), "r"(y) : "memory");
}

__device__ __forceinline__ int uniformize(int v, int bits)
{
    int r = 0;
    for (int k = 0; k < bits; k++) r |= (int)(__ballot_sync(0xffffffffu, (v >> k) & 1) & (1u << k));
    return r;
}

#ifndef NV_CLS_UNROLL
#define NV_CLS_UNROLL 2
#endif
constexpr int CLS_UNROLL = NV_CLS_UNROLL;

__device__ __forceinline__ uint32_t lds_u32(uint32_t addr)
{
    uint32_t v;
    asm("ld.shared.u32 %0, [%1];" : "=r"(v) : "r"(addr));
    return v;
}
__device__ __forceinline__ int rect4(uint32_t wa, const uint4 &o)
{
    return (int)(lds_u32(wa + o.x) - lds_u32(wa + o.y) - lds_u32(wa + o.z) + lds_u32(wa + o.w));
}
__device__ __forceinline__ int nrect4(uint32_t wa, const uint4 &o)
{
    return (int)(lds_u32(wa + o.y) + lds_u32(wa + o.z) - lds_u32(wa + o.x) - lds_u32(wa + o.w));
}
__device__ __forceinline__ void add_if_lt(double &tmp, float f, float thr, double d128)
{
    float m = f < thr ? 1.0f : 0.0f;
    tmp = __fma_rn(d128, __hiloint2double(__float_as_int(m), 0), tmp);
}

template <bool FAST, int NW, typename PT>
__device__ __forceinline__ void class_stage(const PT &P, int si, const uint32_t (&wa)[NW], const float (&vnf)[NW],
                                            bool (&pass)[NW])
{
    const int k0 = P.stage_first[si], k1 = P.stage_first[si + 1];
    const double thr = (double)P.stage_thr[si];
    double tmp[NW];
    if (FAST) {
        const int k6 = P.stage_mid6[si], km = P.stage_mid[si];
#pragma unroll
        for (int i = 0; i < NW; i++) tmp[i] = P.stage_base[si];
#pragma unroll CLS_UNROLL
        for (int k = k0; k < k6; k++) {
            const BulkStump &S = P.s[k];
            const double d = __hiloint2double((int)S.d_hi, (int)S.d_lo);
            const float sthr = __uint_as_float(S.thr);
#pragma unroll
            for (int i = 0; i < NW; i++) {
                int u = (int)(lds_u32(wa[i] + S.o0.x) - lds_u32(wa[i] + S.o0.y));
                int nr0 = (int)(lds_u32(wa[i] + S.o0.z) - lds_u32(wa[i] + S.o0.w)) - u;
                int r1 = u - (int)lds_u32(wa[i] + S.o1.x) + (int)lds_u32(wa[i] + S.o1.y);
                add_if_lt(tmp[i], __fmul_rn(__int2float_rn((int)S.w1 * r1 + nr0), vnf[i]), sthr, d);
            }
        }
#pragma unroll CLS_UNROLL
        for (int k = k6; k < km; k++) {
            const BulkStump &S = P.s[k];
            const double d = __hiloint2double((int)S.d_hi, (int)S.d_lo);
            const float sthr = __uint_as_float(S.thr);
#pragma unroll
            for (int i = 0; i < NW; i++) {
                int r = (int)S.w1 * rect4(wa[i], S.o1) + nrect4(wa[i], S.o0);
                add_if_lt(tmp[i], __fmul_rn(__int2float_rn(r), vnf[i]), sthr, d);
            }
        }
#pragma unroll CLS_UNROLL
        for (int k = km; k < k1; k++) {
            const BulkStump &S = P.s[k];
            const double d = __hiloint2double((int)S.d_hi, (int)S.d_lo);
            const float sthr = __uint_as_float(S.thr);
#pragma unroll
            for (int i = 0; i < NW; i++) {
                int r = (int)S.w1 * rect4(wa[i], S.o1) + (int)S.w2 * rect4(wa[i], P.o2[k]) + nrect4(wa[i], S.o0);
                add_if_lt(tmp[i], __fmul_rn(__int2float_rn(r), vnf[i]), sthr, d);
            }
        }
    } else {
#pragma unroll
        for (int i = 0; i < NW; i++) tmp[i] = 0.;
        for (int k = k0; k < k1; k++) {
            const BulkStump &S = P.s[k];
            const float w0 = __uint_as_float(S.w0), w1 = __uint_as_float(S.w1), w2 = __uint_as_float(S.w2);
            const float sthr = __uint_as_float(S.thr), left = __uint_as_float(S.left), right = __uint_as_float(S.right);
#pragma unroll
            for (int i = 0; i < NW; i++) {
                float f = __fadd_rn(__fmul_rn(w0, __int2float_rn(rect4(wa[i], S.o0))),
                                    __fmul_rn(w1, __int2float_rn(rect4(wa[i], S.o1))));
                if (w2 != 0.f) f = __fadd_rn(f, __fmul_rn(w2, __int2float_rn(rect4(wa[i], P.o2[k]))));
                f = __fmul_rn(f, vnf[i]);
                tmp[i] = __dadd_rn(tmp[i], (double)(f < sthr ? left : right));
            }
        }
    }
#pragma unroll
    for (int i = 0; i < NW; i++) pass[i] = !(tmp[i] < thr);
}

template <int YS, bool FAST>
__global__ void __launch_bounds__(256) k_cascade_classes(const __grid_constant__ TileParams P)
{
    extern __shared__ __align__(128) uint32_t tile[];
    __shared__ __align__(8) unsigned long long mbar;
    __shared__ uint32_t s_mask[3][2][32];
    __shared__ uint32_t s_words[NV_CTY][2];
    const PlanDev *__restrict__ plan = P.plan;
    const int tid = threadIdx.x, lane = tid & 31;
    const int warp = uniformize(tid >> 5, 3);

    int t = blockIdx.x, l = P.level_begin;
    while (l + 1 < P.level_end && plan->lv[l + 1].ctile0 <= t) l++;
    const LevelDesc &L = plan->lv[l];
    int rel = t - L.ctile0, ty = rel / L.cntx, tx = rel - ty * L.cntx;
    int iy0 = ty * NV_CTY, ix0 = tx * NV_CTX;
    const int CP = P.cp, PS = P.ps, K = P.kskew;
    uint32_t bar = smem_u32(&mbar);

    if (tid == 0) mbar_init(bar, 1);
    if (tid < 64) {
        int ly = tid >> 1, cx = 2 * tx + (tid & 1);
        s_words[ly][tid & 1] = (iy0 + ly < L.ny && cx < L.nxw) ? P.bits_alive[L.bofs + (size_t)(iy0 + ly) * L.nxw + cx] : 0u;
    } else {
        (&s_mask[0][0][0])[tid - 64] = 0u;
    }
    __syncthreads();
    if (tid == 0) {
        mbar_expect_tx(bar, (uint32_t)(YS * P.rt * CP * 4));
#pragma unroll
        for (int p = 0; p < YS; p++)
            tma_load_2d(smem_u32(tile + p * PS), P.maps + l, ix0 + p * L.iplane, iy0 * YS, bar);
    }
    {
        uint32_t part = 0;
#pragma unroll
        for (int i = 0; i < 8; i++) {
            int ly = warp * 4 + (i >> 1), h = i & 1;
            uint32_t b = (s_words[ly][h] >> ((lane - K * ly) & 31)) & 1u;
            part |= b << ((ly * 2 + h) & 31);
        }
        if (part) atomicOr(&s_mask[0][warp >> 2][lane], part);
    }
    __syncthreads();
    mbar_wait(bar, 0);

    const uint32_t tile_sa = smem_u32(tile);
    const float *__restrict__ vnf_tile = P.vnf + L.wofs + (size_t)iy0 * L.nx + ix0;
    const int rowb = YS * CP * 4;
    int cur = 0;
    for (int st = P.stage_begin; st < P.stage_end; st++) {
        const int si = st - P.stage_begin;
        uint32_t mlo = s_mask[cur][0][lane], mhi = s_mask[cur][1][lane];
        int maxc = uniformize(__reduce_max_sync(0xffffffffu, __popc(mlo) + __popc(mhi)), 7);
        if (maxc == 0) return;
        int nxt = cur == 2 ? 0 : cur + 1, zer = nxt == 2 ? 0 : nxt + 1;
        if (warp == 0) { s_mask[zer][0][lane] = 0u; s_mask[zer][1][lane] = 0u; }
        unsigned long long rem = ((unsigned long long)mhi << 32) | mlo, pass_bits = 0ull;
        for (int i = 0; i < warp; i++) rem &= rem - 1ull;
        int j = warp;
        for (; j + 8 < maxc; j += 16) {
            int bit[2]; bool active[2], pass[2]; uint32_t wa[2]; float vnf[2]; int ly[2], lx[2];
#pragma unroll
            for (int i = 0; i < 2; i++) {
                active[i] = rem != 0ull;
                bit[i] = active[i] ? __ffsll((long long)rem) - 1 : 0;
                ly[i] = bit[i] >> 1; lx[i] = ((lane - K * ly[i]) & 31) + ((bit[i] & 1) << 5);
                wa[i] = tile_sa + (uint32_t)(ly[i] * rowb + lx[i] * 4);
                vnf[i] = active[i] ? __ldg(vnf_tile + ly[i] * L.nx + lx[i]) : 0.f;
#pragma unroll
                for (int q = 0; q < 8; q++) rem &= rem - 1ull;
            }
            class_stage<FAST, 2>(P, si, wa, vnf, pass);
#pragma unroll
            for (int i = 0; i < 2; i++) {
                if (active[i] && pass[i]) pass_bits |= 1ull << bit[i];
                if (P.depth && active[i] && !pass[i]) P.depth[L.wofs + (iy0 + ly[i]) * L.nx + ix0 + lx[i]] = (int16_t)(-st);
            }
        }
        for (; j < maxc; j += 8) {
            bool active = rem != 0ull;
            int bit = active ? __ffsll((long long)rem) - 1 : 0;
            int ly = bit >> 1, lx = ((lane - K * ly) & 31) + ((bit & 1) << 5);
            uint32_t wa[1] = {tile_sa + (uint32_t)(ly * rowb + lx * 4)};
            float vnf[1] = {active ? __ldg(vnf_tile + ly * L.nx + lx) : 0.f};
            bool pass[1];
            class_stage<FAST, 1>(P, si, wa, vnf, pass);
            if (active && pass[0]) pass_bits |= 1ull << bit;
            if (P.depth && active && !pass[0]) P.depth[L.wofs + (iy0 + ly) * L.nx + ix0 + lx] = (int16_t)(-st);
#pragma unroll
            for (int q = 0; q < 8; q++) rem &= rem - 1ull;
        }
        if ((uint32_t)pass_bits) atomicOr(&s_mask[nxt][0][lane], (uint32_t)pass_bits);
        if ((uint32_t)(pass_bits >> 32)) atomicOr(&s_mask[nxt][1][lane], (uint32_t)(pass_bits >> 32));
        __syncthreads();
        cur = nxt;
    }
    if (warp != 0) return;
    uint32_t mlo = s_mask[cur][0][lane], mhi = s_mask[cur][1][lane];
    int cnt = __popc(mlo) + __popc(mhi), inc = cnt;
#pragma unroll
    for (int d = 1; d < 32; d <<= 1) {
        int v = __shfl_up_sync(0xffffffffu, inc, d);
        if (lane >= d) inc += v;
    }
    int total = __shfl_sync(0xffffffffu, inc, 31);
    if (total == 0) return;
    int *counter = P.counters + (P.final_stage ? 1 : 3);
    int cap = P.final_stage ? P.cand_cap : P.tail_cap;
    int base = 0;
    if (lane == 0) base = atomicAdd(counter, total);
    base = __shfl_sync(0xffffffffu, base, 0) + inc - cnt;
    unsigned long long rem = ((unsigned long long)mhi << 32) | mlo;
    for (; rem; rem &= rem - 1ull, base++) {
        int bit = __ffsll((long long)rem) - 1;
        int ly = bit >> 1, lx = ((lane - K * ly) & 31) + ((bit & 1) << 5);
        uint32_t key = ((uint32_t)l << 26) | ((uint32_t)(iy0 + ly) << 13) | (uint32_t)(ix0 + lx);
        if (base >= cap) { P.counters[2] = 1; continue; }
        if (P.final_stage) {
            P.cand[base] = key;
            if (P.depth) P.depth[L.wofs + (iy0 + ly) * L.nx + ix0 + lx] = NV_DEPTH_PASS;
        } else
            P.tail[base] = make_uint2(key, __float_as_uint(__ldg(vnf_tile + ly * L.nx + lx)));
    }
}

template <int YS, bool FAST, int TW, int TH, int NWARP>
__global__ void __launch_bounds__(32 * NWARP) k_cascade_wide(const __grid_constant__ TileParams P)
{
    constexpr int HW = TW / 32;
    constexpr int NM = TH * HW;
    constexpr int MW = NM / 32;
    constexpr int MPW = NM / NWARP;
    constexpr int NT = 32 * NWARP;
    static_assert(MPW <= 32 && 32 % MPW == 0 && TH % NWARP == 0 && (NWARP == 8 || NWARP == 16), "a warp's rows fill (part of) one mask word");
    extern __shared__ __align__(128) uint32_t tile[];
    __shared__ __align__(8) unsigned long long mbar;
    __shared__ uint32_t s_mask[3][MW][32];
    __shared__ uint32_t s_words[TH][HW];
    const PlanDev *__restrict__ plan = P.plan;
    const int tid = threadIdx.x, lane = tid & 31;
    const int warp = uniformize(tid >> 5, NWARP == 16 ? 4 : 3);

    int t = blockIdx.x, l = P.level_begin;
    while (l + 1 < P.level_end && plan->lv[l + 1].wtile0 <= t) l++;
    const LevelDesc &L = plan->lv[l];
    const int rel = t - L.wtile0, ty = rel / L.wntx, tx = rel - ty * L.wntx;
    const int iy0 = ty * TH, ix0 = tx * TW;
    const int CP = P.cp, PS = P.ps, K = P.kskew;
    const uint32_t bar = smem_u32(&mbar);

    if (tid == 0) mbar_init(bar, 1);
    for (int i = tid; i < TH * HW; i += NT) {
        const int ly = i / HW, h = i - ly * HW, cx = HW * tx + h;
        s_words[ly][h] = (iy0 + ly < L.ny && cx < L.nxw) ? P.bits_alive[L.bofs + (size_t)(iy0 + ly) * L.nxw + cx] : 0u;
    }
    for (int i = tid; i < 3 * MW * 32; i += NT) (&s_mask[0][0][0])[i] = 0u;
    __syncthreads();
    if (tid == 0) {
        mbar_expect_tx(bar, (uint32_t)(YS * P.rt * CP * 4));
#pragma unroll
        for (int p = 0; p < YS; p++)
            tma_load_2d(smem_u32(tile + p * PS), P.maps + l, ix0 + p * L.iplane, iy0 * YS, bar);
    }
    {
        uint32_t part = 0;
#pragma unroll
        for (int i = 0; i < MPW; i++) {
            const int ly = warp * (TH / NWARP) + i / HW, h = i % HW;
            const uint32_t b = (s_words[ly][h] >> ((lane - K * ly) & 31)) & 1u;
            part |= b << i;
        }
        const int m0 = warp * MPW;
        if (part) atomicOr(&s_mask[0][m0 >> 5][lane], part << (m0 & 31));
    }
    __syncthreads();
    mbar_wait(bar, 0);

    const uint32_t tile_sa = smem_u32(tile);
    const float *__restrict__ vnf_tile = P.vnf + L.wofs + (size_t)iy0 * L.nx + ix0;
    const int rowb = YS * CP * 4;
    int cur = 0;
    for (int st = P.stage_begin; st < P.stage_end; st++) {
        const int si = st - P.stage_begin;
        int cnt = 0;
#pragma unroll
        for (int w = 0; w < MW; w++) cnt += __popc(s_mask[cur][w][lane]);
        const int maxc = uniformize(__reduce_max_sync(0xffffffffu, cnt), 9);
        if (maxc == 0) return;
        const int nxt = cur == 2 ? 0 : cur + 1, zer = nxt == 2 ? 0 : nxt + 1;
        if (warp == 0) {
#pragma unroll
            for (int w = 0; w < MW; w++) s_mask[zer][w][lane] = 0u;
        }
        const int q = (maxc + NWARP - 1) / NWARP;
        int skip = warp * q;
        int mine = min(max(cnt - skip, 0), q);
        const int steps = uniformize(min(max(maxc - skip, 0), q), 6);
        int wi = 0;
        uint32_t curw = 0u;
        if (mine > 0) {
            curw = s_mask[cur][0][lane];
            for (int pc = __popc(curw); skip >= pc; pc = __popc(curw)) { skip -= pc; curw = s_mask[cur][++wi][lane]; }
            for (; skip > 0; skip--) curw &= curw - 1u;
        }
        for (int r = 0; r < steps; r += 2) {
            int m[2], ly[2], lx[2]; bool active[2], pass[2]; uint32_t wa[2]; float vnf[2];
#pragma unroll
            for (int i = 0; i < 2; i++) {
                active[i] = mine > 0;
                m[i] = 0;
                if (active[i]) {
                    while (curw == 0u) curw = s_mask[cur][++wi][lane];
                    m[i] = (wi << 5) + __ffs((int)curw) - 1;
                    curw &= curw - 1u;
                    mine--;
                }
                ly[i] = m[i] / HW; lx[i] = ((lane - K * ly[i]) & 31) + ((m[i] % HW) << 5);
                wa[i] = tile_sa + (uint32_t)(ly[i] * rowb + lx[i] * 4);
                vnf[i] = active[i] ? __ldg(vnf_tile + ly[i] * L.nx + lx[i]) : 0.f;
            }
            if (r + 1 < steps) class_stage<FAST, 2>(P, si, wa, vnf, pass);
            else {
                const uint32_t wa1[1] = {wa[0]}; const float vnf1[1] = {vnf[0]}; bool pass1[1];
                class_stage<FAST, 1>(P, si, wa1, vnf1, pass1);
                pass[0] = pass1[0]; pass[1] = false;
            }
#pragma unroll
            for (int i = 0; i < 2; i++) {
                if (active[i] && pass[i]) atomicOr(&s_mask[nxt][m[i] >> 5][lane], 1u << (m[i] & 31));
                if (P.depth && active[i] && !pass[i]) P.depth[L.wofs + (iy0 + ly[i]) * L.nx + ix0 + lx[i]] = (int16_t)(-st);
            }
        }
        __syncthreads();
        cur = nxt;
    }
    if (warp != 0) return;
    int cnt = 0;
#pragma unroll
    for (int w = 0; w < MW; w++) cnt += __popc(s_mask[cur][w][lane]);
    int inc = cnt;
#pragma unroll
    for (int d = 1; d < 32; d <<= 1) {
        int v = __shfl_up_sync(0xffffffffu, inc, d);
        if (lane >= d) inc += v;
    }
    const int total = __shfl_sync(0xffffffffu, inc, 31);
    if (total == 0) return;
    int *counter = P.counters + (P.final_stage ? 1 : 3);
    const int cap = P.final_stage ? P.cand_cap : P.tail_cap;
    int base = 0;
    if (lane == 0) base = atomicAdd(counter, total);
    base = __shfl_sync(0xffffffffu, base, 0) + inc - cnt;
    for (int w = 0; w < MW; w++) {
        for (uint32_t rem = s_mask[cur][w][lane]; rem; rem &= rem - 1u, base++) {
            const int m = (w << 5) + __ffs((int)rem) - 1;
            const int ly = m / HW, lx = ((lane - K * ly) & 31) + ((m % HW) << 5);
            const uint32_t key = ((uint32_t)l << 26) | ((uint32_t)(iy0 + ly) << 13) | (uint32_t)(ix0 + lx);
            if (base >= cap) { P.counters[2] = 1; continue; }
            if (P.final_stage) {
                P.cand[base] = key;
                if (P.depth) P.depth[L.wofs + (iy0 + ly) * L.nx + ix0 + lx] = NV_DEPTH_PASS;
            } else
                P.tail[base] = make_uint2(key, __float_as_uint(__ldg(vnf_tile + ly * L.nx + lx)));
        }
    }
}

template <int YS>
__global__ void __launch_bounds__(256) k_stage0_tiles(const __grid_constant__ Stage0TileParams P)
{
    extern __shared__ __align__(128) uint32_t tile[];
    __shared__ __align__(8) unsigned long long mbar;
    const PlanDev *__restrict__ plan = P.plan;
    const int tid = threadIdx.x, lane = tid & 31;
    const int warp = uniformize(tid >> 5, 3);
    int t = blockIdx.x, l = P.level_begin;
    while (l + 1 < P.level_end && plan->lv[l + 1].ctile0 <= t) l++;
    const LevelDesc &L = plan->lv[l];
    const int rel = t - L.ctile0, ty = rel / L.cntx, tx = rel - ty * L.cntx;
    const int iy0 = ty * NV_CTY, ix0 = tx * NV_CTX;
    const int CP = P.cp, PS = P.ps, K = P.kskew;
    const uint32_t bar = smem_u32(&mbar);
    if (tid == 0) mbar_init(bar, 1);
    __syncthreads();
    if (tid == 0) {
        mbar_expect_tx(bar, (uint32_t)(YS * P.rt * CP * 4));
#pragma unroll
        for (int p = 0; p < YS; p++)
            tma_load_2d(smem_u32(tile + p * PS), P.maps + l, ix0 + p * L.iplane, iy0 * YS, bar);
    }
    const int ww = P.win_w, wh = P.win_h;
    auto gcorner = [&](int dx, int dy) { return dy * L.ipitch + (YS == 2 ? (dx & 1) * L.iplane + (dx >> 1) : dx); };
    const int q00 = gcorner(1, 1), q10 = gcorner(ww - 1, 1), q01 = gcorner(1, wh - 1), q11 = gcorner(ww - 1, wh - 1);
    const uint32_t *__restrict__ sqb = P.sq + L.iofs;
    const double area = (double)((ww - 2) * (wh - 2));
    const uint32_t tile_sa = smem_u32(tile);
    const int rowb = YS * CP * 4;
    mbar_wait(bar, 0);
#pragma unroll 1
    for (int r = 0; r < 4; r++) {
        const int ly = warp * 4 + r, iy = iy0 + ly;
        const int iyc = min(iy, L.ny - 1);
        uint32_t wa[2]; float vnf[2]; bool ok[2], pass[2]; int lx[2];
#pragma unroll
        for (int h = 0; h < 2; h++) {
            lx[h] = ((lane - K * ly) & 31) + (h << 5);
            wa[h] = tile_sa + (uint32_t)(ly * rowb + lx[h] * 4);
            const int ixc = min(ix0 + lx[h], L.nx - 1);
            const uint32_t *qb = sqb + (size_t)iyc * YS * L.ipitch + ixc;
            const int valsum = (int)(lds_u32(wa[h] + P.var.x) - lds_u32(wa[h] + P.var.y) - lds_u32(wa[h] + P.var.z) + lds_u32(wa[h] + P.var.w));
            const uint32_t valsq = __ldg(qb + q00) - __ldg(qb + q10) - __ldg(qb + q01) + __ldg(qb + q11);
            const double nf = __dsub_rn(__dmul_rn(area, (double)valsq), __dmul_rn((double)valsum, (double)valsum));
            vnf[h] = 0.f; ok[h] = false;
            if (nf > 0.) {
                vnf[h] = __double2float_rn(__ddiv_rn(1.0, __dsqrt_rn(nf)));
                ok[h] = __dmul_rn(area, (double)vnf[h]) < 1e-1;
            }
            ok[h] = ok[h] && iy < L.ny && ix0 + lx[h] < L.nx;
        }
        class_stage<true, 2>(P, 0, wa, vnf, pass);
        const int rot = (K * ly) & 31;
#pragma unroll
        for (int h = 0; h < 2; h++) {
            const uint32_t om = __ballot_sync(0xffffffffu, ok[h]), fm = __ballot_sync(0xffffffffu, ok[h] && !pass[h]);
            const int cx = 2 * tx + h;
            if (iy < L.ny && cx < L.nxw) {
                if (lane == 0) {
                    const size_t wi = (size_t)L.bofs + (size_t)iy * L.nxw + cx;
                    P.bits_okv[wi] = __funnelshift_r(om, om, rot);
                    P.bits_fail[wi] = __funnelshift_r(fm, fm, rot);
                }
                if (ok[h]) P.vnf[L.wofs + (size_t)iy * L.nx + ix0 + lx[h]] = vnf[h];
            }
        }
    }
}

struct ChainParams {
    int4 a[NV_MAX_LEVELS];
    int wofs[NV_MAX_LEVELS];
    int nlevels, total_rows;
    const uint32_t *bits_fail, *bits_okv;
    uint32_t *bits_alive;
    int *counters;
    int16_t *depth;
};

__global__ void __launch_bounds__(256) k_stage0_chain(const __grid_constant__ ChainParams P)
{
    const uint32_t *__restrict__ bits_fail = P.bits_fail, *__restrict__ bits_okv = P.bits_okv;
    uint32_t *__restrict__ bits_alive = P.bits_alive;
    int16_t *__restrict__ depth = P.depth;
    int *__restrict__ counters = P.counters;
    const int lane = threadIdx.x & 31;
    const int row = blockIdx.x * 8 + uniformize_s0(threadIdx.x >> 5);
    if (row >= P.total_rows) return;
    int l = 0;
    while (l + 1 < P.nlevels && P.a[l + 1].x <= row) l++;
    struct { int row0, nxw, nx, bofs, wofs; } L = {P.a[l].x, P.a[l].y, P.a[l].z, P.a[l].w, P.wofs[l]};
    const int iy = row - L.row0;
    const size_t wbase = (size_t)L.bofs + (size_t)iy * L.nxw;
    bool carry = true;
    int nalive = 0;
    for (int c0 = 0; c0 < L.nxw; c0 += 32) {
        const int cx = c0 + lane;
        const bool have = cx < L.nxw;
        const uint32_t f = have ? bits_fail[wbase + cx] : 0u, o = have ? bits_okv[wbase + cx] : 0u;
        bool e0 = false, e1 = true;
        const uint32_t em0 = skip_rule_word(f, e0), em1 = skip_rule_word(f, e1);
        bool a = e0, b = e1;
#pragma unroll
        for (int d = 1; d < 32; d <<= 1) {
            const bool pa = __shfl_up_sync(0xffffffffu, (int)a, d), pb = __shfl_up_sync(0xffffffffu, (int)b, d);
            if (lane >= d) { const bool na = pa ? b : a, nb = pb ? b : a; a = na; b = nb; }
        }
        const bool xa = __shfl_up_sync(0xffffffffu, (int)a, 1), xb = __shfl_up_sync(0xffffffffu, (int)b, 1);
        const bool ein = lane == 0 ? carry : (carry ? xb : xa);
        const uint32_t em = ein ? em1 : em0;
        const uint32_t alive = em & o & ~f;
        if (have) bits_alive[wbase + cx] = alive;
        nalive += __popc(alive);
        if (depth && have) {
            for (int j = 0; j < 32; j++) {
                const int ix = cx * 32 + j;
                if (ix < L.nx && !((alive >> j) & 1u))
                    depth[L.wofs + (size_t)iy * L.nx + ix] = (int16_t)(!((em >> j) & 1u) ? NV_DEPTH_SKIPPED : (!((o >> j) & 1u) ? NV_DEPTH_VARREJ : 0));
            }
        }
        const bool la = __shfl_sync(0xffffffffu, (int)a, 31), lb = __shfl_sync(0xffffffffu, (int)b, 31);
        carry = carry ? lb : la;
    }
#pragma unroll
    for (int d = 16; d > 0; d >>= 1) nalive += __shfl_xor_sync(0xffffffffu, nalive, d);
    if (lane == 0 && nalive) atomicAdd(&counters[0], nalive);
}

#define TAIL_MAX_WIN 32
__global__ void __launch_bounds__(256)
k_cascade_tail(const PlanDev *__restrict__ plan, const DevCascade *__restrict__ meta, const DevStump *__restrict__ stumps,
               const uint32_t *__restrict__ sum, const uint2 *__restrict__ tail, int *__restrict__ counters,
               uint32_t *__restrict__ cand, int cand_cap, int16_t *__restrict__ depth, int stage_begin, int order_free)
{
    extern __shared__ uint32_t s_win[];
    int lane = threadIdx.x & 31, warp = threadIdx.x >> 5;
    int n = counters[3], nstages = meta->nstages;
    int ww = plan->win_w, wh = plan->win_h, LP = ww + 1, npatch = (wh + 1) * LP;
    uint32_t *win = s_win + warp * npatch;
    for (;;) {
        int e = 0;
        if (lane == 0) e = atomicAdd(&counters[5], 1);
        e = __shfl_sync(0xffffffffu, e, 0);
        if (e >= n) break;
        uint2 q = tail[e];
        int l = q.x >> 26, iy = (q.x >> 13) & 8191, ix = q.x & 8191;
        float vnf = __uint_as_float(q.y);
        const LevelDesc &L = plan->lv[l];
        const uint32_t *wb = sum + L.iofs + (size_t)iy * L.ystep * L.ipitch + ix;
        __syncwarp();
        for (int idx = lane; idx < npatch; idx += 32) {
            int r = idx / LP, c = idx - r * LP;
            int pc = L.ystep == 2 ? (c & 1) * L.iplane + (c >> 1) : c;
            win[idx] = __ldg(wb + (size_t)r * L.ipitch + pc);
        }
        __syncwarp();
        int code = NV_DEPTH_PASS;
        for (int st = stage_begin; st < nstages; st++) {
            int k0 = meta->stage_first[st], k1 = meta->stage_first[st + 1];
            double tmp = 0.;
            for (int kb = k0; kb < k1; kb += 32) {
                int k = kb + lane;
                double leaf = 0.;
                if (k < k1) {
                    StumpRegs s = load_stump(stumps + k);
                    float f = 0.f;
#pragma unroll
                    for (int j = 0; j < 3; j++) {
                        uint32_t pr = j == 0 ? s.r0 : (j == 1 ? s.r1 : s.r2);
                        float wj = j == 0 ? s.w0 : (j == 1 ? s.w1 : s.w2);
                        if (j == 2 && wj == 0.f) break;
                        int x = pr & 255, y = (pr >> 8) & 255, w = (pr >> 16) & 255, h = pr >> 24;
                        int rs = (int)(win[y * LP + x] - win[y * LP + x + w] - win[(y + h) * LP + x] + win[(y + h) * LP + x + w]);
                        float t = __fmul_rn(wj, __int2float_rn(rs));
                        f = j == 0 ? t : __fadd_rn(f, t);
                    }
                    f = __fmul_rn(f, vnf);
                    leaf = (double)(f < s.thr ? s.left : s.right);
                }
                if (order_free) tmp = __dadd_rn(tmp, leaf);
                else
                    for (int j = 0; j < 32; j++) tmp = __dadd_rn(tmp, __shfl_sync(0xffffffffu, leaf, j));
            }
            if (order_free)
#pragma unroll
                for (int d = 16; d > 0; d >>= 1) tmp = __dadd_rn(tmp, __shfl_xor_sync(0xffffffffu, tmp, d));
            if (tmp < (double)meta->stage_thr[st]) { code = -st; break; }
        }
        if (lane == 0) {
            if (depth) depth[L.wofs + iy * L.nx + ix] = (int16_t)code;
            if (code == NV_DEPTH_PASS) {
                int pos = atomicAdd(&counters[1], 1);
                if (pos < cand_cap) cand[pos] = q.x;
                else counters[2] = 1;
            }
        }
    }
}

#ifdef NV_TAIL_TRACE
__device__ long long g_tail_trace[64 * 16];
__device__ int g_tail_trace_n;
extern "C" __attribute__((visibility("default"))) int nv_debug_tail_trace(long long *out, int cap)
{
    int n = 0;
    cudaMemcpyFromSymbol(&n, g_tail_trace_n, sizeof n);
    cudaMemcpyFromSymbol(out, g_tail_trace, sizeof(long long) * 16 * (n < cap ? n : cap));
    int z = 0;
    cudaMemcpyToSymbol(g_tail_trace_n, &z, sizeof z);
    return n;
}
__device__ __forceinline__ long long clk_after(uint32_t dep)
{
    long long t;
    asm volatile("mov.u64 %0, %%clock64;" : "=l"(t) : "r"(dep));
    return t;
}
#endif
__device__ __forceinline__ void copy_patch(uint32_t *win, const uint32_t *__restrict__ wb, int pitch, int ystep, int iplane, int LP,
                                           int npatch, int lane)
{
    int r = lane / LP, c = lane - r * LP;
    const int dr = 32 / LP, dc = 32 - dr * LP;
    for (int idx = lane; idx < npatch; idx += 128) {
        uint32_t v[4];
#pragma unroll
        for (int u = 0; u < 4; u++) {
            if (idx + 32 * u < npatch) v[u] = __ldg(wb + r * pitch + (ystep == 2 ? (c & 1) * iplane + (c >> 1) : c));
            c += dc; r += dr;
            if (c >= LP) { c -= LP; r++; }
        }
#pragma unroll
        for (int u = 0; u < 4; u++)
            if (idx + 32 * u < npatch) win[idx + 32 * u] = v[u];
    }
}

struct TailRec { uint4 a, b, c; };
__device__ __forceinline__ TailRec load_tail(const TailStump *__restrict__ t, int k)
{
    const uint4 *p = reinterpret_cast<const uint4 *>(t + k);
    return TailRec{__ldg(p), __ldg(p + 1), __ldg(p + 2)};
}

__global__ void __launch_bounds__(256)
k_cascade_tail_fast(const PlanDev *__restrict__ plan, const DevCascade *__restrict__ meta, const TailStump *__restrict__ ts,
                    const double *__restrict__ tbase, const uint32_t *__restrict__ sum, const uint2 *__restrict__ tail,
                    int *__restrict__ counters, uint32_t *__restrict__ cand, int cand_cap, int16_t *__restrict__ depth,
                    int stage_begin, int stage_end, uint2 *__restrict__ deep, int deep_cap)
{
    extern __shared__ uint32_t s_win[];
    const int lane = threadIdx.x & 31, warp = threadIdx.x >> 5;
    const int n = counters[3], nstages = stage_end, nstumps = meta->nstumps;
    const bool last = stage_end == meta->nstages;
    if (!deep) { deep = const_cast<uint2 *>(tail) + n; deep_cap -= n; }
    const int ww = plan->win_w, wh = plan->win_h, LP = ww + 1, npatch = (wh + 1) * LP;
    uint32_t *win = s_win + warp * npatch;
    const uint32_t wsa = smem_u32(win);
    for (;;) {
#ifdef NV_TAIL_TRACE
        long long acc_wait = 0, acc_lds = 0, acc_fp = 0, acc_red = 0, acc_thr = 0, acc_top = 0; int nrounds = 0, nst = 0;
        long long t_begin = clk_after(0);
#endif
        int e = 0;
        if (lane == 0) e = atomicAdd(&counters[5], 1);
        e = __shfl_sync(0xffffffffu, e, 0);
        if (e >= n) break;
        uint2 q = tail[e];
        int l = q.x >> 26, iy = (q.x >> 13) & 8191, ix = q.x & 8191;
        float vnf = __uint_as_float(q.y);
        const LevelDesc &L = plan->lv[l];
        const uint32_t *wb = sum + L.iofs + (size_t)iy * L.ystep * L.ipitch + ix;
        int k0 = meta->stage_first[stage_begin];
        TailRec rec = load_tail(ts, min(k0 + lane, nstumps - 1));
        __syncwarp();
        copy_patch(win, wb, L.ipitch, L.ystep, L.iplane, LP, npatch, lane);
        __syncwarp();
#ifdef NV_TAIL_TRACE
        long long t_copied = clk_after((uint32_t)win[0]);
// ... 252 lines not shown
            }
#pragma unroll
            for (int d = 16; d > 0; d >>= 1) tmp = __dadd_rn(tmp, __shfl_xor_sync(0xffffffffu, tmp, d));
            if (lane == 0) s_part[st & 1][warp] = tmp;
            __syncthreads();
            double total = s_base[st];
#pragma unroll
            for (int w = 0; w < 8; w++) total = __dadd_rn(total, s_part[st & 1][w]);
            k0 = k1;
            if (total < (double)s_thr[st]) { code = -st; break; }
        }
        if (tid == 0) {
            if (depth) depth[L.wofs + iy * L.nx + ix] = (int16_t)code;
            if (code == NV_DEPTH_PASS) {
                const int pos = atomicAdd(&counters[1], 1);
                if (pos < cand_cap) cand[pos] = q.x;
                else counters[2] = 1;
            }
        }
    }
}

void build_tail_stumps(nv_cascade *c)
{
    const DevCascade &m = c->meta;
    bool fast = c->h.order_free != 0 && m.win_w <= 32 && m.win_h <= 32;
    for (int k = 0; k < m.nstumps && fast; k++) {
        const DevStump &d = c->stumps[k];
        double bound = 0;
        for (int j = 0; j < 3; j++) {
            if (d.w[j] != rintf(d.w[j]) || fabsf(d.w[j]) > 4096.f) fast = false;
            bound += fabs((double)d.w[j]) * ((d.r[j] >> 16) & 255) * (d.r[j] >> 24) * 255.0;
        }
        if (bound >= 16777216.0 || d.w[0] != -1.f) fast = false;
    }
    c->tail_fast = fast ? 1 : 0;
    if (!fast) return;
    const int LP = m.win_w + 1;
    c->tail_stumps.clear(); c->tail_base.assign(m.nstages, 0.0);
    for (int s = 0; s < m.nstages; s++) {
        double rsum = 0;
        for (int grp = 0; grp < 2; grp++)
            for (int k = m.stage_first[s]; k < m.stage_first[s + 1]; k++) {
                const DevStump &d = c->stumps[k];
                if ((d.w[2] != 0.f) != (grp == 1)) continue;
                TailStump t;
                memset(&t, 0, sizeof t);
                for (int j = 0; j < 3; j++) {
                    uint32_t r = (j < 2 || d.w[2] != 0.f) ? d.r[j] : d.r[0];
                    int x = r & 255, y = (r >> 8) & 255, w = (r >> 16) & 255, h = r >> 24;
                    t.o[4 * j + 0] = (uint16_t)(4 * (y * LP + x));       t.o[4 * j + 1] = (uint16_t)(4 * (y * LP + x + w));
                    t.o[4 * j + 2] = (uint16_t)(4 * ((y + h) * LP + x)); t.o[4 * j + 3] = (uint16_t)(4 * ((y + h) * LP + x + w));
                }
                t.thr = d.thr; t.w1 = (int16_t)d.w[1]; t.w2 = (int16_t)d.w[2];
                t.d128 = 128.0 * ((double)d.left - (double)d.right);
                rsum += (double)d.right;
                c->tail_stumps.push_back(t);
            }
        c->tail_base[s] = rsum;
    }
}

static void fill_stage_stumps(const nv_cascade *c, int ystep, int cp, int ps, int s, bool fast, BulkStump *S, uint4 *O2, int *n_io,
                              int *mid6, int *mid, double *base)
{
    const DevCascade &m = c->meta;
    auto off = [&](int dx, int dy) { return 4u * (uint32_t)(ystep == 2 ? (dx & 1) * ps + dy * cp + (dx >> 1) : dy * cp + dx); };
    auto f2u = [](float f) { uint32_t u; memcpy(&u, &f, 4); return u; };
    struct Corners {
        uint32_t a, b, c, d;
        bool eq(const Corners &o, int i) const { return i == 0 ? a == o.a : i == 1 ? b == o.b : i == 2 ? c == o.c : d == o.d; }
    };
    auto corners = [&](uint32_t r) {
        int x = r & 255, y = (r >> 8) & 255, w = (r >> 16) & 255, h = r >> 24;
        return Corners{off(x, y), off(x + w, y), off(x, y + h), off(x + w, y + h)};
    };
    auto pattern = [&](const DevStump &d) {
        if (d.w[2] != 0.f) return 0;
        Corners p = corners(d.r[0]), q = corners(d.r[1]);
        bool e[4] = {p.eq(q, 0), p.eq(q, 1), p.eq(q, 2), p.eq(q, 3)};
        if (e[0] && e[2] && !e[1] && !e[3]) return 1;
        if (e[1] && e[3] && !e[0] && !e[2]) return 2;
        if (e[0] && e[1] && !e[2] && !e[3]) return 3;
        if (e[2] && e[3] && !e[0] && !e[1]) return 4;
        return 0;
    };
    int n = *n_io;
    double rsum = 0;
    *mid6 = *mid = n;
    for (int grp = 0; grp < (fast ? 3 : 1); grp++) {
        for (int k = m.stage_first[s]; k < m.stage_first[s + 1]; k++) {
            const DevStump &d = c->stumps[k];
            bool three = d.w[2] != 0.f;
            int pat = pattern(d);
            if (fast && (three ? 2 : (pat ? 0 : 1)) != grp) continue;
            BulkStump &b = S[n];
            Corners p = corners(d.r[0]), q = corners(d.r[1]), t = corners(three ? d.r[2] : d.r[0]);
            b.o0 = make_uint4(p.a, p.b, p.c, p.d); b.o1 = make_uint4(q.a, q.b, q.c, q.d); O2[n] = make_uint4(t.a, t.b, t.c, t.d);
            if (fast && pat == 1) { b.o0 = make_uint4(p.a, p.c, p.b, p.d); b.o1 = make_uint4(q.b, q.d, 0, 0); }
            if (fast && pat == 2) { b.o0 = make_uint4(p.d, p.b, p.c, p.a); b.o1 = make_uint4(q.c, q.a, 0, 0); }
            if (fast && pat == 3) { b.o0 = make_uint4(p.a, p.b, p.c, p.d); b.o1 = make_uint4(q.c, q.d, 0, 0); }
            if (fast && pat == 4) { b.o0 = make_uint4(p.d, p.c, p.b, p.a); b.o1 = make_uint4(q.b, q.a, 0, 0); }
            if (fast) { b.w0 = (uint32_t)(int)d.w[0]; b.w1 = (uint32_t)(int)d.w[1]; b.w2 = (uint32_t)(int)d.w[2]; }
            else { b.w0 = f2u(d.w[0]); b.w1 = f2u(d.w[1]); b.w2 = f2u(d.w[2]); }
            b.thr = f2u(d.thr); b.left = f2u(d.left); b.right = f2u(d.right);
            double dd = 128.0 * ((double)d.left - (double)d.right);
            uint64_t u; memcpy(&u, &dd, 8);
            b.d_lo = (uint32_t)u; b.d_hi = (uint32_t)(u >> 32);
            rsum += (double)d.right;
            n++;
        }
        if (grp == 0 && fast) *mid6 = n;
        if (grp == 1 && fast) *mid = n;
    }
    if (!fast) *mid6 = *mid = *n_io;
    *base = rsum;
    *n_io = n;
}

static bool stages_are_fast(const nv_cascade *c, int stage_begin, int stage_end)
{
    const DevCascade &m = c->meta;
    bool fast = c->h.order_free != 0;
    for (int k = m.stage_first[stage_begin]; k < m.stage_first[stage_end] && fast; k++) {
        const DevStump &d = c->stumps[k];
        double bound = 0;
        for (int j = 0; j < 3; j++) {
            if (d.w[j] != rintf(d.w[j]) || fabsf(d.w[j]) > 4096.f) fast = false;
            bound += fabs((double)d.w[j]) * ((d.r[j] >> 16) & 255) * (d.r[j] >> 24) * 255.0;
        }
        if (bound >= 16777216.0 || d.w[0] != -1.f) fast = false;
    }
    return fast;
}

void fill_bulk_stumps(const nv_cascade *c, int ystep, int cp, int ps, int stage_begin, int stage_end, TileParams *tp)
{
    const DevCascade &m = c->meta;
    tp->stage_begin = stage_begin;
    tp->stage_end = stage_end;
    tp->final_stage = stage_end == m.nstages;
    const bool fast = stages_are_fast(c, stage_begin, stage_end);
    tp->fast = fast ? 1 : 0;
    int n = 0;
    for (int s = stage_begin; s < stage_end; s++) {
        const int si = s - stage_begin;
        tp->stage_first[si] = n;
        tp->stage_thr[si] = m.stage_thr[s];
        fill_stage_stumps(c, ystep, cp, ps, s, fast, tp->s, tp->o2, &n, &tp->stage_mid6[si], &tp->stage_mid[si], &tp->stage_base[si]);
    }
    tp->stage_first[stage_end - stage_begin] = n;
}

bool fill_stage0_tile_params(const nv_cascade *c, int ystep, int cp, int rt, int ps, int kskew, Stage0TileParams *sp)
{
    const DevCascade &m = c->meta;
    const int n0 = m.stage_first[1];
    if (n0 > NV_S0T_MAX_STUMPS || n0 < 1 || !stages_are_fast(c, 0, 1)) return false;
    int n = 0;
    sp->stage_first[0] = 0;
    sp->stage_thr[0] = m.stage_thr[0];
    fill_stage_stumps(c, ystep, cp, ps, 0, true, sp->s, sp->o2, &n, &sp->stage_mid6[0], &sp->stage_mid[0], &sp->stage_base[0]);
    sp->stage_first[1] = n;
    auto off = [&](int dx, int dy) { return 4u * (uint32_t)(ystep == 2 ? (dx & 1) * ps + dy * cp + (dx >> 1) : dy * cp + dx); };
    sp->var = make_uint4(off(1, 1), off(m.win_w - 1, 1), off(1, m.win_h - 1), off(m.win_w - 1, m.win_h - 1));
    sp->win_w = m.win_w; sp->win_h = m.win_h;
    sp->cp = cp; sp->rt = rt; sp->ps = ps; sp->kskew = kskew;
    return true;
}

cudaError_t launch_queue_stages(const PlanDev *plan, const DevCascade *meta, const DevStump *stumps, const uint32_t *sum,
                                const uint2 *queue, int *counters, uint32_t *cand, int cand_cap, int16_t *depth,
                                int nblocks, cudaStream_t st)
{
    k_queue_stages<<<nblocks, 256, 0, st>>>(plan, meta, stumps, sum, queue, counters, cand, cand_cap, depth);
    return cudaGetLastError();
}

cudaError_t launch_stage0_rows(const PlanDev *plan, int total_rows, const DevCascade *meta, const DevStump *stumps,
                               const uint32_t *sum, const uint32_t *sq, float *vnf, uint32_t *bits_alive, int *counters,
                               int16_t *depth, cudaStream_t st)
{
    k_stage0_rows<<<(total_rows + 7) / 8, 256, 0, st>>>(plan, total_rows, meta, stumps, sum, sq, vnf, bits_alive, counters, depth);
    return cudaGetLastError();
}

cudaError_t launch_alive_to_queue(const PlanDev *plan, int total_rows, const float *vnf, const uint32_t *bits_alive,
                                  uint2 *queue, int *counters, int queue_cap, cudaStream_t st, int cidx)
{
    k_alive_to_queue<<<(total_rows + 7) / 8, 256, 0, st>>>(plan, total_rows, vnf, bits_alive, queue, counters, queue_cap, cidx);
    return cudaGetLastError();
}

static cudaError_t raise_smem_limit(const void *kernel, int bytes)
{
    static std::mutex mu;
    static std::set<std::pair<const void *, int>> done;
    int dev = 0;
    cudaError_t e = cudaGetDevice(&dev);
    if (e != cudaSuccess) return e;
    std::lock_guard<std::mutex> lk(mu);
    if (done.count({kernel, dev})) return cudaSuccess;
    if ((e = cudaFuncSetAttribute(kernel, cudaFuncAttributeMaxDynamicSharedMemorySize, bytes)) == cudaSuccess) done.insert({kernel, dev});
    return e;
}

cudaError_t launch_stage0_tiles(const Stage0TileParams &sp, int ystep, int ntiles, cudaStream_t st)
{
    const auto kernel = ystep == 2 ? k_stage0_tiles<2> : k_stage0_tiles<1>;
    cudaError_t e = raise_smem_limit((const void *)kernel, 160 * 1024);
    if (e != cudaSuccess) return e;
    kernel<<<ntiles, 256, (size_t)ystep * sp.ps * sizeof(uint32_t), st>>>(sp);
    return cudaGetLastError();
}

cudaError_t launch_stage0_chain(const PlanDev &plan, const uint32_t *bits_fail, const uint32_t *bits_okv,
                                uint32_t *bits_alive, int *counters, int16_t *depth, cudaStream_t st)
{
    ChainParams cp;
    for (int l = 0; l < plan.nlevels; l++) {
        const LevelDesc &L = plan.lv[l];
        cp.a[l] = make_int4(L.row0, L.nxw, L.nx, L.bofs); cp.wofs[l] = L.wofs;
    }
    cp.nlevels = plan.nlevels; cp.total_rows = plan.total_rows;
    cp.bits_fail = bits_fail; cp.bits_okv = bits_okv; cp.bits_alive = bits_alive; cp.counters = counters; cp.depth = depth;
    k_stage0_chain<<<(plan.total_rows + 7) / 8, 256, 0, st>>>(cp);
    return cudaGetLastError();
}

cudaError_t launch_cascade_classes(const TileParams &tp, int ntiles, cudaStream_t st)
{
    const auto kernel = tp.fast ? k_cascade_classes<2, true> : k_cascade_classes<2, false>;
    cudaError_t e = raise_smem_limit((const void *)kernel, 160 * 1024);
    if (e != cudaSuccess) return e;
    kernel<<<ntiles, 256, 2 * (size_t)tp.ps * sizeof(uint32_t), st>>>(tp);
    return cudaGetLastError();
}

cudaError_t launch_cascade_wide(const TileParams &tp, int ntiles, cudaStream_t st)
{
    const auto kernel = tp.fast ? k_cascade_wide<1, true, NV_WTX, NV_WTY, 8> : k_cascade_wide<1, false, NV_WTX, NV_WTY, 8>;
    cudaError_t e = raise_smem_limit((const void *)kernel, 160 * 1024);
    if (e != cudaSuccess) return e;
    kernel<<<ntiles, 32 * 8, (size_t)tp.ps * sizeof(uint32_t), st>>>(tp);
    return cudaGetLastError();
}

cudaError_t launch_cascade_tail(const PlanDev *plan, const DevCascade *meta, const DevStump *stumps, const uint32_t *sum,
                                const uint2 *tail, int *counters, uint32_t *cand, int cand_cap, int16_t *depth,
                                int stage_begin, int order_free, int nblocks, cudaStream_t st, int smem_bytes)
{
    (void)nblocks;
    k_cascade_tail<<<148 * 8, 256, smem_bytes, st>>>(plan, meta, stumps, sum, tail, counters, cand, cand_cap, depth, stage_begin,
                                                     order_free);
    return cudaGetLastError();
}

cudaError_t launch_cascade_tail_block(const PlanDev *plan, const DevCascade *meta, const TailStump *tstumps, const double *tbase,
                                      const uint32_t *sum, const uint2 *queue, int *counters, int cin, uint32_t *cand, int cand_cap,
                                      int16_t *depth, int stage_begin, int skip_counter, cudaStream_t st)
{
    k_cascade_tail_block<<<148 * 4, 256, 0, st>>>(plan, meta, tstumps, tbase, sum, queue, counters, cin, cand, cand_cap, depth, stage_begin,
                                                 skip_counter);
    return cudaGetLastError();
}

cudaError_t launch_cascade_tail_fast(const PlanDev *plan, const DevCascade *meta, const TailStump *tstumps, const double *tbase,
                                     const uint32_t *sum, const uint2 *tail, int *counters, uint32_t *cand, int cand_cap,
                                     int16_t *depth, int stage_begin, int stage_end, uint2 *deep, int deep_cap, cudaStream_t st,
                                     int smem_bytes)
{
#ifndef NV_TAIL_THREADS
#define NV_TAIL_THREADS 256
#endif
    k_cascade_tail_fast<<<148 * 8 * (256 / NV_TAIL_THREADS), NV_TAIL_THREADS, smem_bytes / (256 / NV_TAIL_THREADS), st>>>(
        plan, meta, tstumps, tbase, sum, tail, counters, cand, cand_cap, depth, stage_begin, stage_end, deep, deep_cap);
    return cudaGetLastError();
}

#ifndef NV_TAILTAB_WARPS
#define NV_TAILTAB_WARPS 8
#endif
size_t tail_tab_smem(const DevCascade &m, int stage_begin, int stage_end)
{
    const size_t nt = (size_t)(m.stage_first[stage_end] - m.stage_first[stage_begin]);
    return nt * 40 + (size_t)NV_TAILTAB_WARPS * (m.win_w + 1) * (m.win_h + 1) * 4;
}

template <bool BATCH>
static cudaError_t launch_tail_tab_t(const PlanDev *plan, const DevCascade *meta, const DevCascade &hmeta, const TailStump *tstumps,
                                     const double *tbase, const uint32_t *sum, const uint2 *tail, int *counters, uint32_t *cand,
                                     int cand_cap, int16_t *depth, int stage_begin, int stage_end, uint2 *deep, int deep_cap,
                                     cudaStream_t st, size_t integ_stride, int cand_stride)
{
    const size_t smem = tail_tab_smem(hmeta, stage_begin, stage_end);
    if (smem > NV_TAILTAB_MAX_SMEM) return cudaErrorInvalidConfiguration;
    cudaError_t e = raise_smem_limit((const void *)k_cascade_tail_tab<NV_TAILTAB_WARPS, BATCH>, (int)NV_TAILTAB_MAX_SMEM);
    if (e != cudaSuccess) return e;
    int per_sm = (int)((227 * 1024) / (smem + 2048));
    per_sm = per_sm < 1 ? 1 : per_sm > 8 ? 8 : per_sm;
    k_cascade_tail_tab<NV_TAILTAB_WARPS, BATCH><<<148 * per_sm, 32 * NV_TAILTAB_WARPS, smem, st>>>(
        plan, meta, tstumps, tbase, sum, tail, counters, cand, cand_cap, depth, stage_begin, stage_end, deep, deep_cap, integ_stride,
        cand_stride);
    return cudaGetLastError();
}

cudaError_t launch_cascade_tail_tab(const PlanDev *plan, const DevCascade *meta, const DevCascade &hmeta, const TailStump *tstumps,
                                    const double *tbase, const uint32_t *sum, const uint2 *tail, int *counters, uint32_t *cand,
                                    int cand_cap, int16_t *depth, int stage_begin, int stage_end, uint2 *deep, int deep_cap,
                                    cudaStream_t st)
{
    return launch_tail_tab_t<false>(plan, meta, hmeta, tstumps, tbase, sum, tail, counters, cand, cand_cap, depth, stage_begin, stage_end,
                                    deep, deep_cap, st, 0, 0);
}

cudaError_t launch_cascade_tail_tab_batch(const PlanDev *plan, const DevCascade *meta, const DevCascade &hmeta, const TailStump *tstumps,
                                          const double *tbase, const uint32_t *sum, size_t integ_stride, const uint2 *queue, int queue_cap,
                                          int *counters, uint32_t *cand, int cand_stride, cudaStream_t st)
{
    return launch_tail_tab_t<true>(plan, meta, hmeta, tstumps, tbase, sum, queue, counters, cand, cand_stride, nullptr, 1, hmeta.nstages,
                                   nullptr, queue_cap, st, integ_stride, cand_stride);
}

cudaError_t launch_stage0_rows_gen(const PlanDev *plan, int total_rows, const DevCascade *meta, const GenModel &g,
                                   const uint32_t *sum, const uint32_t *sq, const uint32_t *tilt, float *vnf,
                                   uint32_t *bits_alive, int *counters, int16_t *depth, cudaStream_t st)
{
    k_stage0_rows_gen<<<(total_rows + 7) / 8, 256, 0, st>>>(plan, total_rows, meta, g, sum, sq, tilt, vnf, bits_alive, counters, depth);
    return cudaGetLastError();
}

cudaError_t launch_queue_stages_gen(const PlanDev *plan, const DevCascade *meta, const GenModel &g, const uint32_t *sum,
                                    const uint32_t *tilt, const uint2 *queue, int *counters, uint32_t *cand, int cand_cap,
                                    int16_t *depth, int nblocks, int order_free, cudaStream_t st)
{
    if (order_free) k_queue_stages_gen_warp<<<nblocks, 256, 0, st>>>(plan, meta, g, sum, tilt, queue, counters, cand, cand_cap, depth, 1, 0);
    else k_queue_stages_gen<<<nblocks, 256, 0, st>>>(plan, meta, g, sum, tilt, queue, counters, cand, cand_cap, depth);
    return cudaGetLastError();
}

cudaError_t launch_queue_stages_gen_staged(const PlanDev *plan, const DevCascade *meta, const GenModel &g, const uint32_t *sum,
                                           const uint32_t *tilt, uint2 *queue_a, uint2 *queue_b, int qcap, int *counters,
                                           uint32_t *cand, int cand_cap, int16_t *depth, int nstages, int order_free,
                                           cudaStream_t st, int *nlaunch)
{
    static const int width[] = {1, 1, 1, 2, 4};
    const int nblocks = 148 * 8;
    uint2 *qin = queue_a, *qout = queue_b;
    int cin = 0, sb = 1, pass = 0;
    for (; pass < 5 && sb < nstages; pass++) {
        const int se = sb + width[pass] < nstages ? sb + width[pass] : nstages;
        const int final = se == nstages;
        k_queue_range_gen<<<nblocks, 256, 0, st>>>(plan, meta, g, sum, tilt, qin, qout, qcap, counters, cin, 8 + pass, cand, cand_cap,
                                                   depth, sb, se, final);
        (*nlaunch)++;
        cin = 8 + pass; sb = se;
        uint2 *t = qin; qin = qout; qout = t;
    }
    if (sb < nstages) {
        if (order_free)
            k_queue_stages_gen_warp<<<nblocks, 256, 0, st>>>(plan, meta, g, sum, tilt, qin, counters, cand, cand_cap, depth, sb, cin);
        else
            k_queue_range_gen<<<nblocks, 256, 0, st>>>(plan, meta, g, sum, tilt, qin, qout, qcap, counters, cin, 15, cand, cand_cap, depth,
                                                       sb, nstages, 1);
        (*nlaunch)++;
    }
    return cudaGetLastError();
}

cudaError_t launch_stage0_rows_p(const Stage0Params &sp, cudaStream_t st)
{
    k_stage0_rows_p<false><<<(sp.total_rows + 7) / 8, 256, 0, st>>>(sp);
    return cudaGetLastError();
}

cudaError_t launch_stage0_rows_p_batch(const Stage0Params &sp, int n, cudaStream_t st)
{
    k_stage0_rows_p<true><<<dim3((sp.total_rows + 7) / 8, n), 256, 0, st>>>(sp);
    return cudaGetLastError();
}
```

Baseline: 2977.

## Fuse stage-0 tile evaluation and skip chain into the cascade tile kernels

Removes the separate stage-0 tile kernels, their fork/join, and the stage-0 chain kernel. Stage 0 (variance normalisation, first-stage stumps, skip-rule chaining) is now evaluated inside the cascade class/wide tile kernels, reusing the integral tile already loaded into shared memory via TMA. Cross-tile ordering of the skip chain is handled with per-row flags and a tick counter using relaxed loads and stores. This saves two launches and the round trip of the fail/ok bit arrays through global memory, but adds inter-block dependencies that can stall tiles waiting on their left neighbours.

```diff
diff --git a/nubomedia-vca_b200/csrc/context.cu b/nubomedia-vca_b200/csrc/context.cu
--- a/nubomedia-vca_b200/csrc/context.cu
+++ b/nubomedia-vca_b200/csrc/context.cu
@@ -265,10 +265,8 @@
         NV_CUDA(cudaStreamCreateWithFlags(&c->stream, cudaStreamNonBlocking));
         NV_CUDA(cudaEventCreateWithFlags(&c->ev_done, cudaEventDisableTiming));
         NV_CUDA(cudaStreamCreateWithFlags(&c->stream2, cudaStreamNonBlocking));
-        for (int i = 0; i < 2; i++) {
-            NV_CUDA(cudaEventCreateWithFlags(&c->ev_fork[i], cudaEventDisableTiming));
-            NV_CUDA(cudaEventCreateWithFlags(&c->ev_join[i], cudaEventDisableTiming));
-        }
+        NV_CUDA(cudaEventCreateWithFlags(&c->ev_fork, cudaEventDisableTiming));
+        NV_CUDA(cudaEventCreateWithFlags(&c->ev_join, cudaEventDisableTiming));
         c->frame_cap = (size_t)max_width * max_height * 4 + 4096;
         NV_CUDA(cudaMallocHost(&c->h_frame, c->frame_cap));
         NV_CUDA(cudaMalloc(&c->d_frame, c->frame_cap));
@@ -305,7 +303,7 @@
     if (c->slots) {
         for (int i = 0; i < NV_PLAN_SLOTS; i++) {
             PlanSlot &sl = c->slots[i];
-            cudaFree(sl.d_plan); cudaFree(sl.d_ptab); cudaFree(sl.d_maps);
+            cudaFree(sl.d_plan); cudaFree(sl.d_ptab); cudaFree(sl.d_maps); cudaFree(sl.d_s0flags);
             if (sl.dexec) cudaGraphExecDestroy(sl.dexec);
         }
         delete[] c->slots;
@@ -320,7 +318,8 @@
     if (c->bexec) cudaGraphExecDestroy(c->bexec);
     batch_free(c->b);
     if (c->ev_done) cudaEventDestroy(c->ev_done);
-    for (int i = 0; i < 2; i++) { if (c->ev_fork[i]) cudaEventDestroy(c->ev_fork[i]); if (c->ev_join[i]) cudaEventDestroy(c->ev_join[i]); }
+    if (c->ev_fork) cudaEventDestroy(c->ev_fork);
+    if (c->ev_join) cudaEventDestroy(c->ev_join);
     if (c->stream2) cudaStreamDestroy(c->stream2);
     for (int i = 0; i <= NV_NUM_STAGES; i++) if (c->prof_ev[i]) cudaEventDestroy(c->prof_ev[i]);
     if (c->stream) cudaStreamDestroy(c->stream);
@@ -549,8 +548,7 @@
         if ((rc = ensure(&ctx->d_vnf, &wcap, (size_t)wofs)) != NV_OK) return rc;
         if ((rc = ensure(&ctx->d_queue, &ctx->queue_cap, (size_t)wofs)) != NV_OK) return rc;
         ctx->win_cap = wcap;
-        if ((rc = ensure(&ctx->d_bits_ok, &ctx->bits_cap, (size_t)bofs * 3)) != NV_OK) return rc;
-        ctx->ps->bits_words = bofs;
+        if ((rc = ensure(&ctx->d_bits_ok, &ctx->bits_cap, (size_t)bofs)) != NV_OK) return rc;
         if (ctx->debug) {
             if ((rc = ensure(&ctx->d_depth, &ctx->depth_cap, (size_t)wofs)) != NV_OK) return rc;
             if ((rc = ensure(&ctx->d_pyr, &ctx->pyr_cap, (size_t)pofs)) != NV_OK) return rc;
@@ -602,49 +600,48 @@
     while (end < m.nstages && end < NV_BULK_MAX_STAGES && m.stage_first[end + 1] - m.stage_first[1] <= NV_BULK_MAX_STUMPS) end++;
     ctx->ps->bulk_end = end;
     static_assert(sizeof(CUtensorMap) == 128, "tensor map size");
-    alignas(64) CUtensorMap maps[2 * NV_MAX_LEVELS];
+    alignas(64) CUtensorMap maps[NV_MAX_LEVELS];
     memset(maps, 0, sizeof maps);
     if (!ctx->ps->d_maps) NV_CUDA(cudaMalloc(&ctx->ps->d_maps, sizeof maps));
     for (int c = 0; c < 2; c++) {
         int ys = c == 0 ? 2 : 1;
         TileParams &tp = ctx->ps->tp[c];
-        struct Geo { int cp, rt, ps, kskew; };
-        auto geometry = [&](int tw, int th) {
-            Geo g;
-            g.cp = align_up(tw + (ys == 2 ? m.win_w / 2 : m.win_w) + 1, 4);
-            if (g.cp % 8 == 0) g.cp += 4;
-            g.rt = (th - 1) * ys + m.win_h + 1;
-            g.kskew = (ys * g.cp) & 31;
-            g.ps = align_up(g.rt * g.cp, 32);
-            return g;
-        };
-        const Geo g0 = geometry(NV_CTX, NV_CTY);
-        const Geo g = ys == 1 ? geometry(NV_WTX, NV_WTY) : g0;
-        if (g.cp > 256 || g.rt > 256) return NV_OK;
-        tp.cp = g.cp; tp.rt = g.rt; tp.kskew = g.kskew; tp.ps = g.ps;
+        const int tw = ys == 1 ? NV_WTX : NV_CTX, th = ys == 1 ? NV_WTY : NV_CTY;
+        tp.cp = align_up(tw + (ys == 2 ? m.win_w / 2 : m.win_w) + 1, 4);
+        if (tp.cp % 8 == 0) tp.cp += 4;
+        tp.rt = (th - 1) * ys + m.win_h + 1;
+        tp.kskew = (ys * tp.cp) & 31;
+        tp.ps = align_up(tp.rt * tp.cp, 32);
+        if (tp.cp > 256 || tp.rt > 256) return NV_OK;
         tp.level_begin = c == 0 ? 0 : P.nlv2;
         tp.level_end = c == 0 ? P.nlv2 : P.nlevels;
         fill_bulk_stumps(casc, ys, tp.cp, tp.ps, 1, end, &tp);
-        Stage0TileParams &s0 = ctx->ps->s0t[c];
-        const bool s0ok = tp.fast && fill_stage0_tile_params(casc, ys, g0.cp, g0.rt, g0.ps, g0.kskew, &s0);
+        const bool s0ok = tp.fast && fill_stage0_bank(casc, ys, tp.cp, tp.ps, &tp.b0);
         ctx->ps->use_s0t = c == 0 ? s0ok : (ctx->ps->use_s0t && s0ok);
-        s0.level_begin = tp.level_begin; s0.level_end = tp.level_end;
+        tp.win_w = m.win_w; tp.win_h = m.win_h;
         for (int l = tp.level_begin; l < tp.level_end; l++) {
             const LevelDesc &L = P.lv[l];
             cuuint64_t gdim[2] = {(cuuint64_t)L.ipitch, (cuuint64_t)(L.lh + 1)};
             cuuint64_t gstr[1] = {(cuuint64_t)L.ipitch * 4};
             cuuint32_t estr[2] = {1, 1};
-            for (int k = 0; k < 2; k++) {
-                cuuint32_t box[2] = {(cuuint32_t)(k == 0 ? g.cp : g0.cp), (cuuint32_t)(k == 0 ? g.rt : g0.rt)};
-                CUresult r = enc(&maps[k * NV_MAX_LEVELS + l], CU_TENSOR_MAP_DATA_TYPE_UINT32, 2, ctx->d_sum + L.iofs, gdim, gstr, box, estr,
-                                 CU_TENSOR_MAP_INTERLEAVE_NONE, CU_TENSOR_MAP_SWIZZLE_NONE, CU_TENSOR_MAP_L2_PROMOTION_L2_128B,
-                                 CU_TENSOR_MAP_FLOAT_OOB_FILL_NONE);
-                if (r != CUDA_SUCCESS) return NV_OK;
-            }
+            cuuint32_t box[2] = {(cuuint32_t)tp.cp, (cuuint32_t)tp.rt};
+            CUresult r = enc(&maps[l], CU_TENSOR_MAP_DATA_TYPE_UINT32, 2, ctx->d_sum + L.iofs, gdim, gstr, box, estr,
+                             CU_TENSOR_MAP_INTERLEAVE_NONE, CU_TENSOR_MAP_SWIZZLE_NONE, CU_TENSOR_MAP_L2_PROMOTION_L2_128B,
+                             CU_TENSOR_MAP_FLOAT_OOB_FILL_NONE);
+            if (r != CUDA_SUCCESS) return NV_OK;
         }
     }
     NV_CUDA(cudaStreamSynchronize(ctx->stream));
     NV_CUDA(cudaMemcpy(ctx->ps->d_maps, maps, sizeof maps, cudaMemcpyHostToDevice));
+    if (ctx->ps->use_s0t) {
+        const size_t f2 = (size_t)P.ctiles2 * NV_CTY, f1 = (size_t)P.wtiles[1] * NV_WTY, words = 4 + f2 + f1;
+        int rc;
+        if ((rc = ensure(&ctx->ps->d_s0flags, &ctx->ps->s0flags_cap, words)) != NV_OK) return rc;
+        NV_CUDA(cudaMemsetAsync(ctx->ps->d_s0flags, 0, words * sizeof(uint32_t), ctx->stream));
+        unsigned long long *tick = reinterpret_cast<unsigned long long *>(ctx->ps->d_s0flags);
+        ctx->ps->tp[0].tick = tick; ctx->ps->tp[0].s0flags = ctx->ps->d_s0flags + 4;
+        ctx->ps->tp[1].tick = tick + 1; ctx->ps->tp[1].s0flags = ctx->ps->d_s0flags + 4 + f2;
+    }
     ctx->ps->use_tiles = true;
     return NV_OK;
 }
@@ -711,25 +708,12 @@
         prof_mark(ctx, 4);
         const bool small_fast = ctx->ps->use_tiles && ctx->cur_tail && P.total_windows <= NV_SMALL_PLAN_WINDOWS && casc->meta.nstages > 1;
         const int qcap = (int)std::min<size_t>(ctx->queue_cap, 0x7fffffff);
+        const bool s0_in_tiles = ctx->ps->use_tiles && ctx->ps->use_s0t && P.total_windows > NV_SMALL_PLAN_WINDOWS;
         bool queued = false;
         if (ctx->use_gen) {
             NV_CUDA(launch_stage0_rows_gen(ctx->ps->d_plan, P.total_rows, meta, ctx->cur_gen, ctx->d_sum, ctx->d_sq, tilt, ctx->d_vnf,
                                            ctx->d_bits_ok, ctx->d_counters, depth, st));
-        } else if (ctx->ps->use_tiles && ctx->ps->use_s0t && P.total_windows > NV_SMALL_PLAN_WINDOWS) {
-            uint32_t *bits_fail = ctx->d_bits_ok + ctx->ps->bits_words, *bits_okv = ctx->d_bits_ok + 2 * (size_t)ctx->ps->bits_words;
-            const bool fork = P.ctiles2 > 0 && P.ctiles1 > 0;
-            if (fork) { NV_CUDA(cudaEventRecord(ctx->ev_fork[0], st)); NV_CUDA(cudaStreamWaitEvent(ctx->stream2, ctx->ev_fork[0], 0)); }
-            for (int c = 0; c < 2; c++) {
-                Stage0TileParams &s0 = ctx->ps->s0t[c];
-                int ntiles = c == 0 ? P.ctiles2 : P.ctiles1;
-                if (ntiles == 0) continue;
-                s0.maps = ctx->ps->d_maps + NV_MAX_LEVELS; s0.plan = ctx->ps->d_plan; s0.sq = ctx->d_sq; s0.vnf = ctx->d_vnf;
-                s0.bits_fail = bits_fail; s0.bits_okv = bits_okv;
-                NV_CUDA(launch_stage0_tiles(s0, c == 0 ? 2 : 1, ntiles, c == 1 && fork ? ctx->stream2 : st));
-                nl++;
-            }
-            if (fork) { NV_CUDA(cudaEventRecord(ctx->ev_join[0], ctx->stream2)); NV_CUDA(cudaStreamWaitEvent(st, ctx->ev_join[0], 0)); }
-            NV_CUDA(launch_stage0_chain(P, bits_fail, bits_okv, ctx->d_bits_ok, ctx->d_counters, depth, st));
+        } else if (s0_in_tiles) {
         } else if (ctx->ps->use_s0p) {
             Stage0Params &sp = ctx->ps->s0p;
             sp.sum = ctx->d_sum; sp.sq = ctx->d_sq; sp.vnf = ctx->d_vnf; sp.bits_alive = ctx->d_bits_ok;
@@ -741,7 +725,7 @@
             NV_CUDA(launch_stage0_rows(ctx->ps->d_plan, P.total_rows, meta, stumps, ctx->d_sum, ctx->d_sq, ctx->d_vnf,
                                        ctx->d_bits_ok, ctx->d_counters, depth, st));
         prof_mark(ctx, 5);
-        nl += 3;
+        nl += s0_in_tiles ? 2 : 3;
         if (small_fast) {
             if (!queued) {
                 NV_CUDA(launch_alive_to_queue(ctx->ps->d_plan, P.total_rows, ctx->d_vnf, ctx->d_bits_ok, ctx->d_queue, ctx->d_counters,
@@ -767,19 +751,20 @@
             }
         } else if (ctx->ps->use_tiles) {
             const bool fork = P.ctiles2 > 0 && P.ctiles1 > 0;
-            if (fork) { NV_CUDA(cudaEventRecord(ctx->ev_fork[1], st)); NV_CUDA(cudaStreamWaitEvent(ctx->stream2, ctx->ev_fork[1], 0)); }
+            if (fork) { NV_CUDA(cudaEventRecord(ctx->ev_fork, st)); NV_CUDA(cudaStreamWaitEvent(ctx->stream2, ctx->ev_fork, 0)); }
             for (int c = 0; c < 2; c++) {
                 TileParams &tp = ctx->ps->tp[c];
                 const cudaStream_t cst = c == 1 && fork ? ctx->stream2 : st;
                 if ((c == 0 ? P.ctiles2 : P.ctiles1) == 0) continue;
                 tp.plan = ctx->ps->d_plan; tp.bits_alive = ctx->d_bits_ok; tp.vnf = ctx->d_vnf; tp.depth = depth;
+                tp.s0 = s0_in_tiles ? 1 : 0; tp.sq = ctx->d_sq;
                 tp.tail = ctx->d_queue; tp.cand = ctx->d_cand; tp.counters = ctx->d_counters; tp.maps = ctx->ps->d_maps;
                 tp.tail_cap = qcap; tp.cand_cap = ctx->cand_cap;
                 if (c == 0) NV_CUDA(launch_cascade_classes(tp, P.ctiles2, cst));
                 else NV_CUDA(launch_cascade_wide(tp, P.wtiles[1], cst));
                 nl++;
             }
-            if (fork) { NV_CUDA(cudaEventRecord(ctx->ev_join[1], ctx->stream2)); NV_CUDA(cudaStreamWaitEvent(st, ctx->ev_join[1], 0)); }
+            if (fork) { NV_CUDA(cudaEventRecord(ctx->ev_join, ctx->stream2)); NV_CUDA(cudaStreamWaitEvent(st, ctx->ev_join, 0)); }
             prof_mark(ctx, 6);
             if (ctx->ps->bulk_end < casc->meta.nstages && ctx->cur_tail) {
                 NV_CUDA(launch_cascade_tail_fast(ctx->ps->d_plan, meta, ctx->cur_tail, ctx->cur_tail_base, ctx->d_sum, ctx->d_queue,
diff --git a/nubomedia-vca_b200/csrc/internal.h b/nubomedia-vca_b200/csrc/internal.h
--- a/nubomedia-vca_b200/csrc/internal.h
+++ b/nubomedia-vca_b200/csrc/internal.h
@@ -167,6 +167,16 @@
     uint32_t left, right;
 };
 
+#define NV_S0T_MAX_STUMPS 8
+struct Stage0Bank {
+    BulkStump s[NV_S0T_MAX_STUMPS];
+    uint4 o2[NV_S0T_MAX_STUMPS];
+    int stage_first[2], stage_mid6[1], stage_mid[1];
+    float stage_thr[1];
+    double stage_base[1];
+    uint4 var;
+};
+
 struct TileParams {
     BulkStump s[NV_BULK_MAX_STUMPS];
     uint4 o2[NV_BULK_MAX_STUMPS];
@@ -184,7 +194,13 @@
     const CUtensorMap *maps;
     const PlanDev *plan;
     const uint32_t *bits_alive;
-    const float *vnf;
+    float *vnf;
+    int s0;
+    int win_w, win_h;
+    Stage0Bank b0;
+    const uint32_t *sq;
+    uint32_t *s0flags;
+    unsigned long long *tick;
     int16_t *depth;
     uint2 *tail;
     uint32_t *cand;
@@ -192,24 +208,6 @@
     int tail_cap, cand_cap;
 };
 static_assert(sizeof(TileParams) <= 32000, "kernel parameter space is 32764 bytes");
-
-#define NV_S0T_MAX_STUMPS 8
-struct Stage0TileParams {
-    BulkStump s[NV_S0T_MAX_STUMPS];
-    uint4 o2[NV_S0T_MAX_STUMPS];
-    int stage_first[2], stage_mid6[1], stage_mid[1];
-    float stage_thr[1];
-    double stage_base[1];
-    uint4 var;
-    int win_w, win_h;
-    int level_begin, level_end;
-    int cp, rt, ps, kskew;
-    const CUtensorMap *maps;
-    const PlanDev *plan;
-    const uint32_t *sq;
-    float *vnf;
-    uint32_t *bits_fail, *bits_okv;
-};
 
 #define NV_S0_MAX_STUMPS 8
 struct Stage0Params {
@@ -252,7 +250,8 @@
     PlanDev plan;
     PlanDev *d_plan = nullptr;
     int *d_ptab = nullptr;       size_t ptab_cap = 0;
-    Stage0TileParams s0t[2];  bool use_s0t = false;  int bits_words = 0;
+    bool use_s0t = false;
+    uint32_t *d_s0flags = nullptr;  size_t s0flags_cap = 0;
     TileParams tp[2];  Stage0Params s0p;  bool use_s0p = false;  CUtensorMap *d_maps = nullptr;  bool use_tiles = false;
     int bulk_end = 0;  unsigned long long tp_casc = 0;  int max_lw = 0;
     unsigned long long last_use = 0, buf_gen = 0;
@@ -270,7 +269,7 @@
     cudaStream_t stream = nullptr;
     cudaEvent_t ev_done = nullptr;
     cudaStream_t stream2 = nullptr;
-    cudaEvent_t ev_fork[2] = {}, ev_join[2] = {};
+    cudaEvent_t ev_fork = nullptr, ev_join = nullptr;
 
     uint8_t *h_frame = nullptr;  size_t frame_cap = 0;
     uint8_t *d_frame = nullptr;
@@ -418,10 +417,7 @@
 cudaError_t launch_alive_to_queue(const PlanDev *plan, int total_rows, const float *vnf, const uint32_t *bits_alive,
                                   uint2 *queue, int *counters, int queue_cap, cudaStream_t st, int cidx = 4);
 void fill_bulk_stumps(const nv_cascade *c, int ystep, int cp, int ps, int stage_begin, int stage_end, TileParams *tp);
-bool fill_stage0_tile_params(const nv_cascade *c, int ystep, int cp, int rt, int ps, int kskew, Stage0TileParams *sp);
-cudaError_t launch_stage0_tiles(const Stage0TileParams &sp, int ystep, int ntiles, cudaStream_t st);
-cudaError_t launch_stage0_chain(const PlanDev &plan, const uint32_t *bits_fail, const uint32_t *bits_okv,
-                                uint32_t *bits_alive, int *counters, int16_t *depth, cudaStream_t st);
+bool fill_stage0_bank(const nv_cascade *c, int ystep, int cp, int ps, Stage0Bank *b);
 void build_tail_stumps(nv_cascade *c);
 cudaError_t launch_cascade_tail_fast(const PlanDev *plan, const DevCascade *meta, const TailStump *tstumps, const double *tbase,
                                      const uint32_t *sum, const uint2 *tail, int *counters, uint32_t *cand, int cand_cap,
diff --git a/nubomedia-vca_b200/csrc/kernels_cascade.cu b/nubomedia-vca_b200/csrc/kernels_cascade.cu
--- a/nubomedia-vca_b200/csrc/kernels_cascade.cu
+++ b/nubomedia-vca_b200/csrc/kernels_cascade.cu
@@ -556,38 +556,188 @@
     for (int i = 0; i < NW; i++) pass[i] = !(tmp[i] < thr);
 }
 
-template <int YS, bool FAST>
+__device__ __forceinline__ uint32_t ld_relaxed(const uint32_t *p)
+{
+    uint32_t v;
+    asm volatile("ld.relaxed.gpu.global.u32 %0, [%1];" : "=r"(v) : "l"(p) : "memory");
+    return v;
+}
+__device__ __forceinline__ void st_relaxed(uint32_t *p, uint32_t v)
+{
+    asm volatile("st.relaxed.gpu.global.u32 [%0], %1;" ::"l"(p), "r"(v) : "memory");
+}
+
+template <bool S0>
+__device__ __forceinline__ float load_vnf(const float *p) { return S0 ? __ldca(p) : __ldg(p); }
+
+template <int YS, int TW, int TH, int NWARP>
+__device__ __forceinline__ void tile_stage0(const TileParams &P, const LevelDesc &L, uint32_t tile_sa, int tile, int tx, int iy0,
+                                            int ix0, uint32_t tag, uint32_t (*s_words)[TW / 32], uint32_t (*s_fail)[TW / 32],
+                                            int warp, int lane)
+{
+    constexpr int HW = TW / 32;
+    const int K = P.kskew, rowb = YS * P.cp * 4;
+    {
+        const int ww = P.win_w, wh = P.win_h;
+        auto gcorner = [&](int dx, int dy) { return dy * L.ipitch + (YS == 2 ? (dx & 1) * L.iplane + (dx >> 1) : dx); };
+        const int q00 = gcorner(1, 1), q10 = gcorner(ww - 1, 1), q01 = gcorner(1, wh - 1), q11 = gcorner(ww - 1, wh - 1);
+        const uint32_t *__restrict__ sqb = P.sq + L.iofs;
+        const double area = (double)((ww - 2) * (wh - 2));
+        constexpr int NR = TH / NWARP * HW / 2;
+        auto sq_corners = [&](int i, uint32_t (&q)[2][4]) {
+            const int ly = warp * (TH / NWARP) + i / (HW / 2), h0 = 2 * (i % (HW / 2));
+            const int iyc = min(iy0 + ly, L.ny - 1);
+#pragma unroll
+            for (int h = 0; h < 2; h++) {
+                const int ixc = min(ix0 + ((lane - K * ly) & 31) + ((h0 + h) << 5), L.nx - 1);
+                const uint32_t *qb = sqb + (size_t)iyc * YS * L.ipitch + ixc;
+                q[h][0] = __ldg(qb + q00); q[h][1] = __ldg(qb + q10); q[h][2] = __ldg(qb + q01); q[h][3] = __ldg(qb + q11);
+            }
+        };
+        uint32_t qn[2][4];
+        sq_corners(0, qn);
+#pragma unroll 1
+        for (int i = 0; i < NR; i++) {
+            const int ly = warp * (TH / NWARP) + i / (HW / 2), h0 = 2 * (i % (HW / 2)), iy = iy0 + ly;
+            uint32_t q[2][4];
+#pragma unroll
+            for (int h = 0; h < 2; h++)
+#pragma unroll
+                for (int j = 0; j < 4; j++) q[h][j] = qn[h][j];
+            if (i + 1 < NR) sq_corners(i + 1, qn);
+            uint32_t wa[2]; float vnf[2]; bool ok[2], pass[2]; int lx[2];
+#pragma unroll
+            for (int h = 0; h < 2; h++) {
+                lx[h] = ((lane - K * ly) & 31) + ((h0 + h) << 5);
+                wa[h] = tile_sa + (uint32_t)(ly * rowb + lx[h] * 4);
+                const int valsum = (int)(lds_u32(wa[h] + P.b0.var.x) - lds_u32(wa[h] + P.b0.var.y) - lds_u32(wa[h] + P.b0.var.z) +
+                                         lds_u32(wa[h] + P.b0.var.w));
+                const uint32_t valsq = q[h][0] - q[h][1] - q[h][2] + q[h][3];
+                const double nf = __dsub_rn(__dmul_rn(area, (double)valsq), __dmul_rn((double)valsum, (double)valsum));
+                vnf[h] = 0.f; ok[h] = false;
+                if (nf > 0.) {
+                    vnf[h] = __double2float_rn(__ddiv_rn(1.0, __dsqrt_rn(nf)));
+                    ok[h] = __dmul_rn(area, (double)vnf[h]) < 1e-1;
+                }
+                ok[h] = ok[h] && iy < L.ny && ix0 + lx[h] < L.nx;
+            }
+            class_stage<true, 2>(P.b0, 0, wa, vnf, pass);
+            const int rot = (K * ly) & 31;
+#pragma unroll
+            for (int h = 0; h < 2; h++) {
+                const uint32_t om = __ballot_sync(0xffffffffu, ok[h]), fm = __ballot_sync(0xffffffffu, ok[h] && !pass[h]);
+                if (lane == 0) { s_words[ly][h0 + h] = __funnelshift_r(om, om, rot); s_fail[ly][h0 + h] = __funnelshift_r(fm, fm, rot); }
+                if (ok[h]) P.vnf[L.wofs + (size_t)iy * L.nx + ix0 + lx[h]] = vnf[h];
+            }
+        }
+    }
+    __syncthreads();
+    if (warp < TH / 32) {
+        const int ly = warp * 32 + lane;
+        uint32_t okw[HW], fw[HW];
+        bool o0 = false, o1 = true;
+#pragma unroll
+        for (int h = 0; h < HW; h++) {
+            okw[h] = s_words[ly][h]; fw[h] = s_fail[ly][h];
+            skip_rule_word(fw[h], o0); skip_rule_word(fw[h], o1);
+        }
+        uint32_t *flag = P.s0flags + (size_t)tile * TH + ly;
+        bool cin = true;
+        if (tx == 0) st_relaxed(flag, tag | 4u | (o1 ? 1u : 0u));
+        else {
+            st_relaxed(flag, tag | (o0 ? 1u : 0u) | (o1 ? 2u : 0u));
+            bool g0 = false, g1 = true;
+            for (const uint32_t *q = flag - TH;; q -= TH) {
+                uint32_t w = ld_relaxed(q);
+                while ((w & ~7u) != tag) { __nanosleep(64); w = ld_relaxed(q); }
+                if (w & 4u) { cin = (w & 1u) ? g1 : g0; break; }
+                const bool n0 = (w & 1u) ? g1 : g0, n1 = (w & 2u) ? g1 : g0;
+                g0 = n0; g1 = n1;
+                if (g0 == g1) { cin = g0; break; }
+            }
+            st_relaxed(flag, tag | 4u | ((cin ? o1 : o0) ? 1u : 0u));
+        }
+        uint32_t vis[HW], alive[HW];
+        int nalive = 0;
+#pragma unroll
+        for (int h = 0; h < HW; h++) {
+            vis[h] = skip_rule_word(fw[h], cin);
+            alive[h] = vis[h] & okw[h] & ~fw[h];
+            s_words[ly][h] = alive[h];
+            nalive += __popc(alive[h]);
+        }
+#pragma unroll
+        for (int d = 16; d > 0; d >>= 1) nalive += __shfl_xor_sync(0xffffffffu, nalive, d);
+        if (lane == 0 && nalive) atomicAdd(&P.counters[0], nalive);
+        if (P.depth) {
+#pragma unroll 1
+            for (int r = 0; r < 32; r++) {
+                const int iy = iy0 + warp * 32 + r;
+#pragma unroll
+                for (int h = 0; h < HW; h++) {
+                    const uint32_t a = __shfl_sync(0xffffffffu, alive[h], r), v = __shfl_sync(0xffffffffu, vis[h], r),
+                                   o = __shfl_sync(0xffffffffu, okw[h], r);
+                    const int ix = ix0 + (h << 5) + lane;
+                    if (iy < L.ny && ix < L.nx && !((a >> lane) & 1u))
+                        P.depth[L.wofs + (size_t)iy * L.nx + ix] =
+                            (int16_t)(!((v >> lane) & 1u) ? NV_DEPTH_SKIPPED : (!((o >> lane) & 1u) ? NV_DEPTH_VARREJ : 0));
+                }
+            }
+        }
+    }
+    __syncthreads();
+}
+
+template <int YS, bool FAST, bool S0>
 __global__ void __launch_bounds__(256) k_cascade_classes(const __grid_constant__ TileParams P)
 {
+    static_assert(FAST || !S0, "stage 0 on the tile needs the certificates");
     extern __shared__ __align__(128) uint32_t tile[];
     __shared__ __align__(8) unsigned long long mbar;
+    __shared__ unsigned long long s_ticket;
     __shared__ uint32_t s_mask[3][2][32];
     __shared__ uint32_t s_words[NV_CTY][2];
     const PlanDev *__restrict__ plan = P.plan;
     const int tid = threadIdx.x, lane = tid & 31;
     const int warp = uniformize(tid >> 5, 3);
-
-    int t = blockIdx.x, l = P.level_begin;
+    uint32_t bar = smem_u32(&mbar);
+
+    int t = blockIdx.x;
+    uint32_t tag = 0;
+    if (S0) {
+        if (tid == 0) { mbar_init(bar, 1); s_ticket = atomicAdd(P.tick, 1ull); }
+        else if (tid <= 128) (&s_mask[0][0][0])[tid - 1] = 0u;
+        __syncthreads();
+        t = (int)(s_ticket % gridDim.x);
+        tag = (uint32_t)(s_ticket / gridDim.x + 1) << 3;
+    }
+    int l = P.level_begin;
     while (l + 1 < P.level_end && plan->lv[l + 1].ctile0 <= t) l++;
     const LevelDesc &L = plan->lv[l];
     int rel = t - L.ctile0, ty = rel / L.cntx, tx = rel - ty * L.cntx;
     int iy0 = ty * NV_CTY, ix0 = tx * NV_CTX;
     const int CP = P.cp, PS = P.ps, K = P.kskew;
-    uint32_t bar = smem_u32(&mbar);
-
-    if (tid == 0) mbar_init(bar, 1);
-    if (tid < 64) {
-        int ly = tid >> 1, cx = 2 * tx + (tid & 1);
-        s_words[ly][tid & 1] = (iy0 + ly < L.ny && cx < L.nxw) ? P.bits_alive[L.bofs + (size_t)(iy0 + ly) * L.nxw + cx] : 0u;
-    } else {
-        (&s_mask[0][0][0])[tid - 64] = 0u;
-    }
-    __syncthreads();
+
+    if (!S0) {
+        if (tid == 0) mbar_init(bar, 1);
+        if (tid < 64) {
+            int ly = tid >> 1, cx = 2 * tx + (tid & 1);
+            s_words[ly][tid & 1] = (iy0 + ly < L.ny && cx < L.nxw) ? P.bits_alive[L.bofs + (size_t)(iy0 + ly) * L.nxw + cx] : 0u;
+        } else {
+            (&s_mask[0][0][0])[tid - 64] = 0u;
+        }
+        __syncthreads();
+    }
     if (tid == 0) {
         mbar_expect_tx(bar, (uint32_t)(YS * P.rt * CP * 4));
 #pragma unroll
         for (int p = 0; p < YS; p++)
             tma_load_2d(smem_u32(tile + p * PS), P.maps + l, ix0 + p * L.iplane, iy0 * YS, bar);
+    }
+    if (S0) {
+        mbar_wait(bar, 0);
+        tile_stage0<YS, NV_CTX, NV_CTY, 8>(P, L, smem_u32(tile), t, tx, iy0, ix0, tag, s_words,
+                                            reinterpret_cast<uint32_t (*)[2]>(&s_mask[2][0][0]), warp, lane);
     }
     {
         uint32_t part = 0;
@@ -600,7 +750,7 @@
         if (part) atomicOr(&s_mask[0][warp >> 2][lane], part);
     }
     __syncthreads();
-    mbar_wait(bar, 0);
+    if (!S0) mbar_wait(bar, 0);
 
     const uint32_t tile_sa = smem_u32(tile);
     const float *__restrict__ vnf_tile = P.vnf + L.wofs + (size_t)iy0 * L.nx + ix0;
@@ -624,7 +774,7 @@
                 bit[i] = active[i] ? __ffsll((long long)rem) - 1 : 0;
                 ly[i] = bit[i] >> 1; lx[i] = ((lane - K * ly[i]) & 31) + ((bit[i] & 1) << 5);
                 wa[i] = tile_sa + (uint32_t)(ly[i] * rowb + lx[i] * 4);
-                vnf[i] = active[i] ? __ldg(vnf_tile + ly[i] * L.nx + lx[i]) : 0.f;
+                vnf[i] = active[i] ? load_vnf<S0>(vnf_tile + ly[i] * L.nx + lx[i]) : 0.f;
 #pragma unroll
                 for (int q = 0; q < 8; q++) rem &= rem - 1ull;
             }
@@ -640,7 +790,7 @@
             int bit = active ? __ffsll((long long)rem) - 1 : 0;
             int ly = bit >> 1, lx = ((lane - K * ly) & 31) + ((bit & 1) << 5);
             uint32_t wa[1] = {tile_sa + (uint32_t)(ly * rowb + lx * 4)};
-            float vnf[1] = {active ? __ldg(vnf_tile + ly * L.nx + lx) : 0.f};
+            float vnf[1] = {active ? load_vnf<S0>(vnf_tile + ly * L.nx + lx) : 0.f};
             bool pass[1];
             class_stage<FAST, 1>(P, si, wa, vnf, pass);
             if (active && pass[0]) pass_bits |= 1ull << bit;
@@ -678,11 +828,11 @@
             P.cand[base] = key;
             if (P.depth) P.depth[L.wofs + (iy0 + ly) * L.nx + ix0 + lx] = NV_DEPTH_PASS;
         } else
-            P.tail[base] = make_uint2(key, __float_as_uint(__ldg(vnf_tile + ly * L.nx + lx)));
-    }
-}
-
-template <int YS, bool FAST, int TW, int TH, int NWARP>
+            P.tail[base] = make_uint2(key, __float_as_uint(load_vnf<S0>(vnf_tile + ly * L.nx + lx)));
+    }
+}
+
+template <int YS, bool FAST, int TW, int TH, int NWARP, bool S0>
 __global__ void __launch_bounds__(32 * NWARP) k_cascade_wide(const __grid_constant__ TileParams P)
 {
     constexpr int HW = TW / 32;
@@ -691,34 +841,53 @@
     constexpr int MPW = NM / NWARP;
     constexpr int NT = 32 * NWARP;
     static_assert(MPW <= 32 && 32 % MPW == 0 && TH % NWARP == 0 && (NWARP == 8 || NWARP == 16), "a warp's rows fill (part of) one mask word");
+    static_assert(FAST || !S0, "stage 0 on the tile needs the certificates");
+    static_assert(!S0 || (TH % 32 == 0 && HW % 2 == 0 && TH / 32 <= NWARP), "tile_stage0: a warp per 32 rows, two words a round");
     extern __shared__ __align__(128) uint32_t tile[];
     __shared__ __align__(8) unsigned long long mbar;
+    __shared__ unsigned long long s_ticket;
     __shared__ uint32_t s_mask[3][MW][32];
     __shared__ uint32_t s_words[TH][HW];
     const PlanDev *__restrict__ plan = P.plan;
     const int tid = threadIdx.x, lane = tid & 31;
     const int warp = uniformize(tid >> 5, NWARP == 16 ? 4 : 3);
-
-    int t = blockIdx.x, l = P.level_begin;
+    const uint32_t bar = smem_u32(&mbar);
+
+    int t = blockIdx.x;
+    uint32_t tag = 0;
+    if (S0) {
+        if (tid == 0) { mbar_init(bar, 1); s_ticket = atomicAdd(P.tick, 1ull); }
+        for (int i = tid; i < 2 * MW * 32; i += NT) (&s_mask[0][0][0])[i] = 0u;
+        __syncthreads();
+        t = (int)(s_ticket % gridDim.x);
+        tag = (uint32_t)(s_ticket / gridDim.x + 1) << 3;
+    }
+    int l = P.level_begin;
     while (l + 1 < P.level_end && plan->lv[l + 1].wtile0 <= t) l++;
     const LevelDesc &L = plan->lv[l];
     const int rel = t - L.wtile0, ty = rel / L.wntx, tx = rel - ty * L.wntx;
     const int iy0 = ty * TH, ix0 = tx * TW;
     const int CP = P.cp, PS = P.ps, K = P.kskew;
-    const uint32_t bar = smem_u32(&mbar);
-
-    if (tid == 0) mbar_init(bar, 1);
-    for (int i = tid; i < TH * HW; i += NT) {
-        const int ly = i / HW, h = i - ly * HW, cx = HW * tx + h;
-        s_words[ly][h] = (iy0 + ly < L.ny && cx < L.nxw) ? P.bits_alive[L.bofs + (size_t)(iy0 + ly) * L.nxw + cx] : 0u;
-    }
-    for (int i = tid; i < 3 * MW * 32; i += NT) (&s_mask[0][0][0])[i] = 0u;
-    __syncthreads();
+
+    if (!S0) {
+        if (tid == 0) mbar_init(bar, 1);
+        for (int i = tid; i < TH * HW; i += NT) {
+            const int ly = i / HW, h = i - ly * HW, cx = HW * tx + h;
+            s_words[ly][h] = (iy0 + ly < L.ny && cx < L.nxw) ? P.bits_alive[L.bofs + (size_t)(iy0 + ly) * L.nxw + cx] : 0u;
+        }
+        for (int i = tid; i < 3 * MW * 32; i += NT) (&s_mask[0][0][0])[i] = 0u;
+        __syncthreads();
+    }
     if (tid == 0) {
         mbar_expect_tx(bar, (uint32_t)(YS * P.rt * CP * 4));
 #pragma unroll
         for (int p = 0; p < YS; p++)
             tma_load_2d(smem_u32(tile + p * PS), P.maps + l, ix0 + p * L.iplane, iy0 * YS, bar);
+    }
+    if (S0) {
+        mbar_wait(bar, 0);
+        tile_stage0<YS, TW, TH, NWARP>(P, L, smem_u32(tile), t, tx, iy0, ix0, tag, s_words,
+                                       reinterpret_cast<uint32_t (*)[HW]>(&s_mask[2][0][0]), warp, lane);
     }
     {
         uint32_t part = 0;
@@ -732,7 +901,7 @@
         if (part) atomicOr(&s_mask[0][m0 >> 5][lane], part << (m0 & 31));
     }
     __syncthreads();
-    mbar_wait(bar, 0);
+    if (!S0) mbar_wait(bar, 0);
 
     const uint32_t tile_sa = smem_u32(tile);
     const float *__restrict__ vnf_tile = P.vnf + L.wofs + (size_t)iy0 * L.nx + ix0;
@@ -775,7 +944,7 @@
                 }
                 ly[i] = m[i] / HW; lx[i] = ((lane - K * ly[i]) & 31) + ((m[i] % HW) << 5);
                 wa[i] = tile_sa + (uint32_t)(ly[i] * rowb + lx[i] * 4);
-                vnf[i] = active[i] ? __ldg(vnf_tile + ly[i] * L.nx + lx[i]) : 0.f;
+                vnf[i] = active[i] ? load_vnf<S0>(vnf_tile + ly[i] * L.nx + lx[i]) : 0.f;
             }
             if (r + 1 < steps) class_stage<FAST, 2>(P, si, wa, vnf, pass);
             else {
@@ -819,138 +988,9 @@
                 P.cand[base] = key;
                 if (P.depth) P.depth[L.wofs + (iy0 + ly) * L.nx + ix0 + lx] = NV_DEPTH_PASS;
             } else
-                P.tail[base] = make_uint2(key, __float_as_uint(__ldg(vnf_tile + ly * L.nx + lx)));
-        }
-    }
-}
-
-template <int YS>
-__global__ void __launch_bounds__(256) k_stage0_tiles(const __grid_constant__ Stage0TileParams P)
-{
-    extern __shared__ __align__(128) uint32_t tile[];
-    __shared__ __align__(8) unsigned long long mbar;
-    const PlanDev *__restrict__ plan = P.plan;
-    const int tid = threadIdx.x, lane = tid & 31;
-    const int warp = uniformize(tid >> 5, 3);
-    int t = blockIdx.x, l = P.level_begin;
-    while (l + 1 < P.level_end && plan->lv[l + 1].ctile0 <= t) l++;
-    const LevelDesc &L = plan->lv[l];
-    const int rel = t - L.ctile0, ty = rel / L.cntx, tx = rel - ty * L.cntx;
-    const int iy0 = ty * NV_CTY, ix0 = tx * NV_CTX;
-    const int CP = P.cp, PS = P.ps, K = P.kskew;
-    const uint32_t bar = smem_u32(&mbar);
-    if (tid == 0) mbar_init(bar, 1);
-    __syncthreads();
-    if (tid == 0) {
-        mbar_expect_tx(bar, (uint32_t)(YS * P.rt * CP * 4));
-#pragma unroll
-        for (int p = 0; p < YS; p++)
-            tma_load_2d(smem_u32(tile + p * PS), P.maps + l, ix0 + p * L.iplane, iy0 * YS, bar);
-    }
-    const int ww = P.win_w, wh = P.win_h;
-    auto gcorner = [&](int dx, int dy) { return dy * L.ipitch + (YS == 2 ? (dx & 1) * L.iplane + (dx >> 1) : dx); };
-    const int q00 = gcorner(1, 1), q10 = gcorner(ww - 1, 1), q01 = gcorner(1, wh - 1), q11 = gcorner(ww - 1, wh - 1);
-    const uint32_t *__restrict__ sqb = P.sq + L.iofs;
-    const double area = (double)((ww - 2) * (wh - 2));
-    const uint32_t tile_sa = smem_u32(tile);
-    const int rowb = YS * CP * 4;
-    mbar_wait(bar, 0);
-#pragma unroll 1
-    for (int r = 0; r < 4; r++) {
-        const int ly = warp * 4 + r, iy = iy0 + ly;
-        const int iyc = min(iy, L.ny - 1);
-        uint32_t wa[2]; float vnf[2]; bool ok[2], pass[2]; int lx[2];
-#pragma unroll
-        for (int h = 0; h < 2; h++) {
-            lx[h] = ((lane - K * ly) & 31) + (h << 5);
-            wa[h] = tile_sa + (uint32_t)(ly * rowb + lx[h] * 4);
-            const int ixc = min(ix0 + lx[h], L.nx - 1);
-            const uint32_t *qb = sqb + (size_t)iyc * YS * L.ipitch + ixc;
-            const int valsum = (int)(lds_u32(wa[h] + P.var.x) - lds_u32(wa[h] + P.var.y) - lds_u32(wa[h] + P.var.z) + lds_u32(wa[h] + P.var.w));
-            const uint32_t valsq = __ldg(qb + q00) - __ldg(qb + q10) - __ldg(qb + q01) + __ldg(qb + q11);
-            const double nf = __dsub_rn(__dmul_rn(area, (double)valsq), __dmul_rn((double)valsum, (double)valsum));
-            vnf[h] = 0.f; ok[h] = false;
-            if (nf > 0.) {
-                vnf[h] = __double2float_rn(__ddiv_rn(1.0, __dsqrt_rn(nf)));
-                ok[h] = __dmul_rn(area, (double)vnf[h]) < 1e-1;
-            }
-            ok[h] = ok[h] && iy < L.ny && ix0 + lx[h] < L.nx;
-        }
-        class_stage<true, 2>(P, 0, wa, vnf, pass);
-        const int rot = (K * ly) & 31;
-#pragma unroll
-        for (int h = 0; h < 2; h++) {
-            const uint32_t om = __ballot_sync(0xffffffffu, ok[h]), fm = __ballot_sync(0xffffffffu, ok[h] && !pass[h]);
-            const int cx = 2 * tx + h;
-            if (iy < L.ny && cx < L.nxw) {
-                if (lane == 0) {
-                    const size_t wi = (size_t)L.bofs + (size_t)iy * L.nxw + cx;
-                    P.bits_okv[wi] = __funnelshift_r(om, om, rot);
-                    P.bits_fail[wi] = __funnelshift_r(fm, fm, rot);
-                }
-                if (ok[h]) P.vnf[L.wofs + (size_t)iy * L.nx + ix0 + lx[h]] = vnf[h];
-            }
-        }
-    }
-}
-
-struct ChainParams {
-    int4 a[NV_MAX_LEVELS];
-    int wofs[NV_MAX_LEVELS];
-    int nlevels, total_rows;
-    const uint32_t *bits_fail, *bits_okv;
-    uint32_t *bits_alive;
-    int *counters;
-    int16_t *depth;
-};
-
-__global__ void __launch_bounds__(256) k_stage0_chain(const __grid_constant__ ChainParams P)
-{
-    const uint32_t *__restrict__ bits_fail = P.bits_fail, *__restrict__ bits_okv = P.bits_okv;
-    uint32_t *__restrict__ bits_alive = P.bits_alive;
-    int16_t *__restrict__ depth = P.depth;
-    int *__restrict__ counters = P.counters;
-    const int lane = threadIdx.x & 31;
-    const int row = blockIdx.x * 8 + uniformize_s0(threadIdx.x >> 5);
-    if (row >= P.total_rows) return;
-    int l = 0;
-    while (l + 1 < P.nlevels && P.a[l + 1].x <= row) l++;
-    struct { int row0, nxw, nx, bofs, wofs; } L = {P.a[l].x, P.a[l].y, P.a[l].z, P.a[l].w, P.wofs[l]};
-    const int iy = row - L.row0;
-    const size_t wbase = (size_t)L.bofs + (size_t)iy * L.nxw;
-    bool carry = true;
-    int nalive = 0;
-    for (int c0 = 0; c0 < L.nxw; c0 += 32) {
-        const int cx = c0 + lane;
-        const bool have = cx < L.nxw;
-        const uint32_t f = have ? bits_fail[wbase + cx] : 0u, o = have ? bits_okv[wbase + cx] : 0u;
-        bool e0 = false, e1 = true;
-        const uint32_t em0 = skip_rule_word(f, e0), em1 = skip_rule_word(f, e1);
-        bool a = e0, b = e1;
-#pragma unroll
-        for (int d = 1; d < 32; d <<= 1) {
-            const bool pa = __shfl_up_sync(0xffffffffu, (int)a, d), pb = __shfl_up_sync(0xffffffffu, (int)b, d);
-            if (lane >= d) { const bool na = pa ? b : a, nb = pb ? b : a; a = na; b = nb; }
-        }
-        const bool xa = __shfl_up_sync(0xffffffffu, (int)a, 1), xb = __shfl_up_sync(0xffffffffu, (int)b, 1);
-        const bool ein = lane == 0 ? carry : (carry ? xb : xa);
-        const uint32_t em = ein ? em1 : em0;
-        const uint32_t alive = em & o & ~f;
-        if (have) bits_alive[wbase + cx] = alive;
-        nalive += __popc(alive);
-        if (depth && have) {
-            for (int j = 0; j < 32; j++) {
-                const int ix = cx * 32 + j;
-                if (ix < L.nx && !((alive >> j) & 1u))
-                    depth[L.wofs + (size_t)iy * L.nx + ix] = (int16_t)(!((em >> j) & 1u) ? NV_DEPTH_SKIPPED : (!((o >> j) & 1u) ? NV_DEPTH_VARREJ : 0));
-            }
-        }
-        const bool la = __shfl_sync(0xffffffffu, (int)a, 31), lb = __shfl_sync(0xffffffffu, (int)b, 31);
-        carry = carry ? lb : la;
-    }
-#pragma unroll
-    for (int d = 16; d > 0; d >>= 1) nalive += __shfl_xor_sync(0xffffffffu, nalive, d);
-    if (lane == 0 && nalive) atomicAdd(&counters[0], nalive);
+                P.tail[base] = make_uint2(key, __float_as_uint(load_vnf<S0>(vnf_tile + ly * L.nx + lx)));
+        }
+    }
 }
 
 #define TAIL_MAX_WIN 32
@@ -1509,20 +1549,18 @@
     tp->stage_first[stage_end - stage_begin] = n;
 }
 
-bool fill_stage0_tile_params(const nv_cascade *c, int ystep, int cp, int rt, int ps, int kskew, Stage0TileParams *sp)
+bool fill_stage0_bank(const nv_cascade *c, int ystep, int cp, int ps, Stage0Bank *b)
 {
     const DevCascade &m = c->meta;
     const int n0 = m.stage_first[1];
     if (n0 > NV_S0T_MAX_STUMPS || n0 < 1 || !stages_are_fast(c, 0, 1)) return false;
     int n = 0;
-    sp->stage_first[0] = 0;
-    sp->stage_thr[0] = m.stage_thr[0];
-    fill_stage_stumps(c, ystep, cp, ps, 0, true, sp->s, sp->o2, &n, &sp->stage_mid6[0], &sp->stage_mid[0], &sp->stage_base[0]);
-    sp->stage_first[1] = n;
+    b->stage_first[0] = 0;
+    b->stage_thr[0] = m.stage_thr[0];
+    fill_stage_stumps(c, ystep, cp, ps, 0, true, b->s, b->o2, &n, &b->stage_mid6[0], &b->stage_mid[0], &b->stage_base[0]);
+    b->stage_first[1] = n;
     auto off = [&](int dx, int dy) { return 4u * (uint32_t)(ystep == 2 ? (dx & 1) * ps + dy * cp + (dx >> 1) : dy * cp + dx); };
-    sp->var = make_uint4(off(1, 1), off(m.win_w - 1, 1), off(1, m.win_h - 1), off(m.win_w - 1, m.win_h - 1));
-    sp->win_w = m.win_w; sp->win_h = m.win_h;
-    sp->cp = cp; sp->rt = rt; sp->ps = ps; sp->kskew = kskew;
+    b->var = make_uint4(off(1, 1), off(m.win_w - 1, 1), off(1, m.win_h - 1), off(m.win_w - 1, m.win_h - 1));
     return true;
 }
 
@@ -1562,32 +1600,9 @@
     return e;
 }
 
-cudaError_t launch_stage0_tiles(const Stage0TileParams &sp, int ystep, int ntiles, cudaStream_t st)
-{
-    const auto kernel = ystep == 2 ? k_stage0_tiles<2> : k_stage0_tiles<1>;
-    cudaError_t e = raise_smem_limit((const void *)kernel, 160 * 1024);
-    if (e != cudaSuccess) return e;
-    kernel<<<ntiles, 256, (size_t)ystep * sp.ps * sizeof(uint32_t), st>>>(sp);
-    return cudaGetLastError();
-}
-
-cudaError_t launch_stage0_chain(const PlanDev &plan, const uint32_t *bits_fail, const uint32_t *bits_okv,
-                                uint32_t *bits_alive, int *counters, int16_t *depth, cudaStream_t st)
-{
-    ChainParams cp;
-    for (int l = 0; l < plan.nlevels; l++) {
-        const LevelDesc &L = plan.lv[l];
-        cp.a[l] = make_int4(L.row0, L.nxw, L.nx, L.bofs); cp.wofs[l] = L.wofs;
-    }
-    cp.nlevels = plan.nlevels; cp.total_rows = plan.total_rows;
-    cp.bits_fail = bits_fail; cp.bits_okv = bits_okv; cp.bits_alive = bits_alive; cp.counters = counters; cp.depth = depth;
-    k_stage0_chain<<<(plan.total_rows + 7) / 8, 256, 0, st>>>(cp);
-    return cudaGetLastError();
-}
-
 cudaError_t launch_cascade_classes(const TileParams &tp, int ntiles, cudaStream_t st)
 {
-    const auto kernel = tp.fast ? k_cascade_classes<2, true> : k_cascade_classes<2, false>;
+    const auto kernel = tp.s0 ? k_cascade_classes<2, true, true> : tp.fast ? k_cascade_classes<2, true, false> : k_cascade_classes<2, false, false>;
     cudaError_t e = raise_smem_limit((const void *)kernel, 160 * 1024);
     if (e != cudaSuccess) return e;
     kernel<<<ntiles, 256, 2 * (size_t)tp.ps * sizeof(uint32_t), st>>>(tp);
@@ -1596,7 +1611,9 @@
 
 cudaError_t launch_cascade_wide(const TileParams &tp, int ntiles, cudaStream_t st)
 {
-    const auto kernel = tp.fast ? k_cascade_wide<1, true, NV_WTX, NV_WTY, 8> : k_cascade_wide<1, false, NV_WTX, NV_WTY, 8>;
+    const auto kernel = tp.s0     ? k_cascade_wide<1, true, NV_WTX, NV_WTY, 8, true>
+                        : tp.fast ? k_cascade_wide<1, true, NV_WTX, NV_WTY, 8, false>
+                                  : k_cascade_wide<1, false, NV_WTX, NV_WTY, 8, false>;
     cudaError_t e = raise_smem_limit((const void *)kernel, 160 * 1024);
     if (e != cudaSuccess) return e;
     kernel<<<ntiles, 32 * 8, (size_t)tp.ps * sizeof(uint32_t), st>>>(tp);
```

Result: no change. 2967 (median of 6 runs) (-0.3%).
